# AIBluefisher/DReg-NeRF

Hardware: AMD Instinct MI355X
Metric: nerf_pairs_per_sec_regtr_fwd_bwd_128 (higher is better)
Workload: dtype bf16; 1 GPU; RegTR fwd+bwd+AdamW, shell-R synthetic pairs, 128^3 grids, 4 pairs (8 grids) per GPU per step, random-init weights; global_batch_pairs=4, resolution=128, fpn_head=active-set (identical results; rows around occupied voxels), parallelism=dp1

## Files before the change

dreg_nerf_amd/csrc/executor.hip:

```cpp
#include <hip/hip_runtime.h>
#include <cstdint>
#include <cstring>
#include <algorithm>
#include <vector>
#include <string>
#include <cstdio>
#include "../../include/dreg_nerf.h"
#ifndef DREG_ELAUNCH
#define DREG_ELAUNCH (-2)
#endif

namespace {

enum { OP_CONV = 0, OP_BN = 1, OP_MAXPOOL = 2, OP_CONV_ROWS = 3 };
constexpr int OP_INTS = 16;
constexpr int TENSOR_INTS = 5;
constexpr int RL = 8;
constexpr int PARAM_I64 = 5;

struct Tensor { int B, D, H, W, C; size_t bytes, off, goff; };
struct Param {
    float* val; float* grad; int d0, d1, ksz;
    size_t pk_fwd = SIZE_MAX, pk_dgrad = SIZE_MAX, pk_cls = SIZE_MAX;
    size_t pk_halo_fwd = SIZE_MAX, pk_halo_dgrad = SIZE_MAX;
    size_t pk_brick_fwd = SIZE_MAX, pk_brick_dgrad = SIZE_MAX;
    int cin_pad = 0;
};
struct Op {
    int kind, in, out, in2, w, b, p2, p3, p4, ksz, stride, pad, relu, add_same, rows_out, rows_in;
    size_t aux0 = 0, aux1 = 0;
    size_t wg_off = 0, wg_bytes = 0;
    int rd = -1;
    int ds_rows = -1;
    int sparse_gx = 0;
    size_t cl_off = 0;
    int cl_count = 0;
    int ds_sparse = 0;
    size_t cl2_off = 0;
    int cl2_count = 0;
    int pool = -1;
    int sstem = 0;
    int sstem_conv = -1, sstem_lat = -1;
    size_t xam_off = 0, pmask_off = 0;
    int halo = 0;
    int pointwise = 0;
    int stats_bn = -1;
    size_t stats_off = 0;
    int stats_conv = -1;
    int grp = 0;
    int fold_sk_fwd = 0, fold_sk_bwd = 0;
    int fold_into = -1, res_from = -1;
    int bt = -1;
    size_t keep_var = 0, keep_sums = 0;
};
struct HaloPack { const float* w; size_t off; int Cout, Cin, transposed, brick; };
struct PackRec { const float* w; void* out; int Cout, Cin_real, inner, ntaps, for_dgrad, Kpad, dtype, row0; };
static_assert(sizeof(PackRec) == 48, "matches PackDesc of conv.hip");

struct ReduceRec { const float* part; float* dw; int nsplit, Cout, Kpad, ntaps, Cin, Cin_real, accumulate, block0; };
static_assert(sizeof(ReduceRec) == 48, "matches WgradReduceDesc of conv.hip");

struct BnTailRec { const float* a; const float* b; float* o0; float* o1; int B, V, C, block0; };
static_assert(sizeof(BnTailRec) == 48, "matches BnTailDesc of fpn_ops.hip");

struct TimedLaunch { hipEvent_t e0, e1; int op, kind, variant; };

struct Exec {
    std::vector<Tensor> t;
    std::vector<Op> ops;
    std::vector<Param> prm;
    std::vector<char> needs_grad;
    size_t act_bytes = 0, arena_bytes = 0, pack_bytes = 0;
    size_t off_bn_ws = 0, off_coef = 0, off_ks = 0, off_rd = 0, off_cs = 0, off_tmp = 0;
    size_t sz_ks = 0;
    std::vector<ReduceRec> reduce;
    const void* sparse_arena = nullptr;
    std::vector<ReduceRec> reduce_abs;
    int reduce_blocks = 0;
    const void* reduce_arena = nullptr;
    std::vector<BnTailRec> bn_fwd, bn_bwd;
    size_t off_bnf = 0, off_bnb = 0;
    int bn_blocks = 0;
    std::vector<PackRec> packs;
    std::vector<HaloPack> halo_packs;
    int pack_rows = 0, pack_max_floats = 0;
    int out_slot = -1;
    bool timing = false;
    std::vector<TimedLaunch> timed;
    size_t timed_used = 0;
    hipStream_t aux = nullptr;
    std::vector<hipEvent_t> ev;
    hipEvent_t ev_done = nullptr;
    bool use_aux = true;
    const uint8_t* in_rowocc = nullptr;
    char* pack_base = nullptr;
    std::vector<char> written;
    bool aux_used = false;
    struct GrpLaunch { size_t off; int n, variant, blocks; };
    std::vector<int> grp_ops;
    std::vector<GrpLaunch> grp_launch;
    size_t off_grp = 0;
    bool grp_ready = false;
    int pend_sk_bn = -1, pend_sk_n = 0;
    size_t pend_sk_slice = 0;
    const void* fwd_rows_arena = nullptr;
    struct Band { size_t off; const char* tag; int idx; };
    std::vector<Band> bands;
    size_t off_guard_tab = 0, off_guard_res = 0;
    const void* guard_arena = nullptr;
    int guard_op = -1, guard_pass = 0; long long guard_band = -1;
    dreg_exec_opts opt;
};

inline size_t align256(size_t v) { return (v + 255) / 256 * 256; }
constexpr size_t GUARD_BYTES = 64 * 1024;
struct Bump {
    size_t v = 0;
    std::vector<Exec::Band>* bands = nullptr;
    const char* tag = "?"; int idx = -1;
    operator size_t() const { return v; }
    Bump& operator+=(size_t n) { v += n; if (bands && n) { bands->push_back(Exec::Band{v, tag, idx}); v += GUARD_BYTES; } return *this; }
    void name(const char* t, int i) { tag = t; idx = i; }
};
inline int out_dim(int i, int k, int s, int p) { return (i + 2 * p - k) / s + 1; }

struct Scope {
    Exec* e; hipStream_t st; TimedLaunch* tl = nullptr;
    Scope(Exec* ex, hipStream_t s, int op, int kind) : e(ex), st(s) {
        if (!e->timing) return;
        if (e->timed_used == e->timed.size()) {
            TimedLaunch n{}; n.op = op; n.kind = kind;
            if (hipEventCreate(&n.e0) != hipSuccess || hipEventCreate(&n.e1) != hipSuccess) return;
            e->timed.push_back(n);
        }
        tl = &e->timed[e->timed_used++];
        tl->op = op; tl->kind = kind; tl->variant = 0;
        (void)hipEventRecord(tl->e0, st);
    }
    ~Scope() { if (tl) (void)hipEventRecord(tl->e1, st); }
    void variant(int v) { if (tl) tl->variant = v; }
};

#define CK(expr) do { int rc_ = (expr); if (rc_) return rc_; } while (0)

bool s2_class_ok(const Param& p, int ksz, int stride, int pad)
{
    return stride == 2 && ((ksz == 3 && pad == 1) || (ksz == 1 && pad == 0)) && p.d0 % 64 == 0 && p.d1 % 64 == 0 && dreg_conv_get_glds();
}

}

extern "C" {

void dreg_exec_default_opts(dreg_exec_opts* o)
{
    std::memset(o, 0, sizeof(*o));
    o->sparse_grads = 1; o->bn_batch_tails = 1; o->fuse_stem = 1; o->sparse_stem = 1; o->fold_res_bn = 1; o->fold_splitk = 1;
    o->group_wgrad = 1; o->s2_accumulate = 1; o->fuse_bn_stats = 1; o->brick = 1; o->defer_head_pg = 0; o->pointwise_stream = 1;
}
void* dreg_exec_create(const int* tensors, int nt, const int* ops, int nops, const int64_t* params, int np)
{
    return dreg_exec_create_opts(tensors, nt, ops, nops, params, np, nullptr);
}
void* dreg_exec_create_opts(const int* tensors, int nt, const int* ops, int nops, const int64_t* params, int np, const dreg_exec_opts* opts)
{
    Exec* e = new Exec();
    if (opts) e->opt = *opts; else dreg_exec_default_opts(&e->opt);
    e->opt.brick &= 3;
    const int g_sparse_grads = e->opt.sparse_grads, g_bn_batch_tails = e->opt.bn_batch_tails, g_fuse_stem = e->opt.fuse_stem, g_sparse_stem = e->opt.sparse_stem,
              g_fold_res_bn = e->opt.fold_res_bn, g_fold_splitk = e->opt.fold_splitk, g_group_wgrad = e->opt.group_wgrad, g_fuse_bn_stats = e->opt.fuse_bn_stats,
              g_brick = e->opt.brick;
    e->t.resize(nt);
    for (int i = 0; i < nt; ++i) {
        Tensor& t = e->t[i];
        t.B = tensors[i * TENSOR_INTS]; t.D = tensors[i * TENSOR_INTS + 1]; t.H = tensors[i * TENSOR_INTS + 2];
        t.W = tensors[i * TENSOR_INTS + 3]; t.C = tensors[i * TENSOR_INTS + 4];
        t.bytes = align256((size_t)t.B * t.D * t.H * t.W * t.C * 2);
    }
    e->prm.resize(np);
    for (int i = 0; i < np; ++i) {
        Param& p = e->prm[i];
        p.val = (float*)params[i * PARAM_I64]; p.grad = (float*)params[i * PARAM_I64 + 1];
        p.d0 = (int)params[i * PARAM_I64 + 2]; p.d1 = (int)params[i * PARAM_I64 + 3]; p.ksz = (int)params[i * PARAM_I64 + 4];
    }
    e->ops.resize(nops);
    for (int i = 0; i < nops; ++i) {
        const int* r = ops + i * OP_INTS;
        Op& o = e->ops[i];
        o.kind = r[0]; o.in = r[1]; o.out = r[2]; o.in2 = r[3]; o.w = r[4]; o.b = r[5]; o.p2 = r[6]; o.p3 = r[7]; o.p4 = r[8];
        o.ksz = r[9]; o.stride = r[10]; o.pad = r[11]; o.relu = r[12]; o.add_same = r[13]; o.rows_out = r[14]; o.rows_in = r[15];
        if (o.in < 0 || o.in >= nt || o.out <= 0 || o.out >= nt || o.in2 >= nt) { delete e; return nullptr; }
    }
    e->out_slot = nops ? e->ops.back().out : -1;

    e->needs_grad.assign(nt, 0);
    for (const Op& o : e->ops) {
        bool g = e->needs_grad[o.in] || (o.in2 >= 0 && e->needs_grad[o.in2]);
        if (o.kind == OP_CONV || o.kind == OP_CONV_ROWS) g = g || e->prm[o.w].grad || (o.b >= 0 && e->prm[o.b].grad);
        if (o.kind == OP_BN) g = g || e->prm[o.w].grad || e->prm[o.b].grad;
        e->needs_grad[o.out] = g;
    }

    for (size_t i = 0; i + 1 < e->ops.size(); ++i) {
        Op& o = e->ops[i];
        if (o.kind != OP_BN || o.in2 >= 0 || o.out == e->out_slot) continue;
        int users = 0, pool = -1;
        for (size_t j = 0; j < e->ops.size(); ++j) {
            const Op& q = e->ops[j];
            if (q.in == o.out || q.in2 == o.out) { ++users; if (q.kind == OP_MAXPOOL && q.in == o.out && j > i) pool = (int)j; }
        }
        if (users == 1 && pool >= 0 && e->t[o.out].C % 8 == 0 && g_fuse_stem) { o.pool = pool; e->ops[pool].pool = (int)i; }
        if (o.pool < 0 && pool >= 0 && o.relu && e->t[o.out].C % 8 == 0 && g_sparse_stem && g_fuse_stem) {
            int prod = -1, writers = 0, lat = -1, others = 0;
            for (size_t j = 0; j < e->ops.size(); ++j) {
                const Op& q = e->ops[j];
                if (q.out == o.in) { prod = (int)j; ++writers; }
                if ((int)j == pool) continue;
                if (q.in2 == o.out) ++others;
                else if (q.in == o.out) { if (q.kind == OP_CONV_ROWS && q.rows_in >= 0 && lat < 0) lat = (int)j; else ++others; }
            }
            if (writers == 1 && others == 0 && e->ops[prod].kind == OP_CONV && e->ops[prod].rows_out >= 0 && o.b >= 0) {
                o.pool = pool; e->ops[pool].pool = (int)i; o.sstem = 1; o.sstem_conv = prod; o.sstem_lat = lat;
            }
        }
// ... 10 lines not shown
                if (o.in == bj.out) ++users;
                if (o.in2 == bj.out) { ++users; if (o.kind == OP_BN && q > j && o.pool < 0) k = (int)q; }
            }
            if (users != 1 || k < 0 || e->ops[k].res_from >= 0) continue;
            bj.fold_into = k; e->ops[k].res_from = (int)j;
        }

    if (g_fold_splitk)
        for (size_t i = 0; i < e->ops.size(); ++i) {
            Op& o = e->ops[i];
            if (o.kind != OP_CONV || o.b >= 0 || o.in2 >= 0 || o.relu || o.rows_out >= 0) continue;
            auto users = [&](int slot) { int u = 0; for (const Op& q : e->ops) u += (q.in == slot) + (q.in2 == slot); return u; };
            const Tensor& y = e->t[o.out];
            if (i + 1 < e->ops.size() && o.out != e->out_slot) {
                const Op& bn = e->ops[i + 1];
                if (bn.kind == OP_BN && bn.in == o.out && bn.pool < 0 && users(o.out) == 1 && dreg_bn_small_in_regs(y.B, y.D * y.H * y.W, y.C, 0)) o.fold_sk_fwd = 1;
            }
            const Tensor& x = e->t[o.in];
            if (i >= 1 && o.in != 0) {
                const Op& bn = e->ops[i - 1];
                if (bn.kind == OP_BN && bn.out == o.in && bn.pool < 0 && users(o.in) == 1 && dreg_bn_small_in_regs(x.B, x.D * x.H * x.W, x.C, 0) && o.stride == 1) o.fold_sk_bwd = 1;
            }
        }

    Bump off;
    if (e->opt.guard) { off.bands = &e->bands; off.name("arena start", 0); off += 256; }
    for (int i = 1; i < nt; ++i) { off.name("activation", i); e->t[i].off = off; off += e->t[i].bytes; }
    size_t max_tensor = 0, bn_ws = 0, coef = 0, cs = 0;
    for (Op& o : e->ops) {
        const Tensor& x = e->t[o.in];
        off.name(o.kind == OP_BN ? "BatchNorm statistics / stem scratch of op" : (o.kind == OP_MAXPOOL ? "max-pool argmax of op" : "conv op"), (int)(&o - e->ops.data()));
        if (o.kind == OP_BN) {
            const size_t sb = align256((size_t)x.B * x.C * 2 * sizeof(float));
            o.aux0 = off; off += sb; o.aux1 = off; off += sb;
            const size_t V = (size_t)x.D * x.H * x.W;
            size_t w = (size_t)x.B * dreg_bn_num_chunks((int)V) * x.C * 2 * sizeof(float);
            if (o.sstem) {
                const Tensor& p = e->t[e->ops[o.pool].out];
                const size_t w2 = dreg_sparse_stem_workspace_floats(p.B, p.D, p.H, p.W, p.C) * sizeof(float);
                if (w2 > w) w = w2;
                o.xam_off = off; off += align256((size_t)p.B * p.D * p.H * p.W * p.C * 2);
                o.pmask_off = off; off += align256((size_t)p.B * p.D * p.H * p.W);
            }
            if (w > bn_ws) bn_ws = w;
            if (sb > coef) coef = sb;
            bool shared = false;
            for (const Op& q : e->ops) shared = shared || (&q != &o && q.kind == OP_BN && (q.w == o.w || q.b == o.b || q.p2 == o.p2 || q.p3 == o.p3));
            if (g_bn_batch_tails && o.pool < 0 && !shared && dreg_bn_small(x.B, (int)V, x.C, 0)) {
                o.keep_var = off; off += align256((size_t)x.B * x.C * sizeof(float));
                o.keep_sums = off; off += sb;
                BnTailRec f{}, b{};
                f.a = (const float*)o.aux1; f.b = (const float*)o.keep_var; f.o0 = e->prm[o.p2].val; f.o1 = e->prm[o.p3].val;
                b.a = (const float*)o.keep_sums; b.b = nullptr; b.o0 = e->prm[o.w].grad; b.o1 = e->prm[o.b].grad;
                f.B = b.B = x.B; f.V = b.V = (int)V; f.C = b.C = x.C; f.block0 = b.block0 = e->bn_blocks;
                e->bn_blocks += (x.C + 255) / 256;
                o.bt = (int)e->bn_fwd.size();
                e->bn_fwd.push_back(f); e->bn_bwd.push_back(b);
            }
        } else if (o.kind == OP_MAXPOOL) {
            const Tensor& y = e->t[o.out];
            o.aux0 = off; off += align256((size_t)y.B * y.D * y.H * y.W * y.C);
        } else {
            const Param& w = e->prm[o.w];
            const Tensor& y = e->t[o.out];
            const size_t k1 = dreg_conv3d_igemm_workspace_bytes(x.B, x.D, x.H, x.W, x.C, y.D, y.H, y.W, w.d0, o.ksz, o.stride, o.pad, 0, o.in2 >= 0, 0);
            const size_t k2 = dreg_conv3d_igemm_workspace_bytes(x.B, y.D, y.H, y.W, w.d0, x.D, x.H, x.W, w.d1, o.ksz, o.stride, o.pad, 1, 0, 0);
            if (k1 > e->sz_ks) e->sz_ks = k1;
            if (k2 > e->sz_ks) e->sz_ks = k2;
            if (w.grad) {
                o.wg_bytes = dreg_conv3d_wgrad_workspace_bytes(x.B, y.D, y.H, y.W, x.C, w.d0, o.ksz, 0);
                bool shared = false;
                for (const ReduceRec& q : e->reduce) shared = shared || q.dw == w.grad;
                if (shared) o.rd = -2;
                else {
                    ReduceRec r{};
                    r.dw = w.grad; r.nsplit = dreg_conv3d_wgrad_splits(x.B, y.D, y.H, y.W, x.C, w.d0, o.ksz, 0);
                    r.Cout = w.d0; r.Kpad = dreg_conv3d_kpad(o.ksz, x.C, 0); r.ntaps = o.ksz * o.ksz * o.ksz; r.Cin = x.C; r.Cin_real = w.d1;
                    r.accumulate = (o.kind == OP_CONV_ROWS || o.rows_out >= 0) ? 3 : 1;
                    r.block0 = e->reduce_blocks;
                    e->reduce_blocks += dreg_wgrad_reduce_blocks(w.d0, w.d1, o.ksz, r.nsplit);
                    o.rd = (int)e->reduce.size();
                    e->reduce.push_back(r);
                }
            }
            const size_t c = dreg_colsum_workspace_bytes((size_t)y.B * y.D * y.H * y.W, w.d0);
            if (c > cs) cs = c;
        }
    }
    if (g_fuse_bn_stats) {
        for (size_t j = 0; j < e->ops.size(); ++j) {
            Op& bn = e->ops[j];
            if (bn.kind != OP_BN || bn.pool >= 0) continue;
            const Tensor& x = e->t[bn.in];
            const int V = x.D * x.H * x.W;
            if (V % 128 != 0 || dreg_bn_small(x.B, V, x.C, 0)) continue;
            int prod = -1, writers = 0;
            for (size_t i = 0; i < j; ++i) if (e->ops[i].out == bn.in) { prod = (int)i; ++writers; }
            if (writers != 1 || e->ops[prod].kind != OP_CONV || e->ops[prod].stats_bn >= 0) continue;
            {
                const Op& pc = e->ops[prod];
                const Tensor& px = e->t[pc.in];
                const Param& pp = e->prm[pc.w];
                if (!pc.relu && pp.d1 == px.C && pp.d0 != 64 && dreg_conv3_halo_use(px.B, px.D, px.H, px.W, px.C, pp.d0, pc.ksz, pc.stride, pc.pad)) continue;
            }
            e->ops[prod].stats_bn = (int)j;
            bn.stats_conv = prod;
// ... 128 lines not shown
        if (o.halo & 1) { if (p.pk_halo_fwd == SIZE_MAX) p.pk_halo_fwd = add_halo_pack(p, 0); }
        else if (p.pk_fwd == SIZE_MAX) { p.cin_pad = x.C; p.pk_fwd = add_pack(p, 0, x.C); }
        if (e->needs_grad[o.in]) {
            if (o.halo & 2) { if (p.pk_halo_dgrad == SIZE_MAX) p.pk_halo_dgrad = add_halo_pack(p, 1); }
            else if (o.kind == OP_CONV && s2_class_ok(p, o.ksz, o.stride, o.pad)) { if (p.pk_cls == SIZE_MAX) p.pk_cls = add_pack(p, 2, x.C); }
            else if (p.pk_dgrad == SIZE_MAX) p.pk_dgrad = add_pack(p, 1, x.C);
        }
    }
    e->pack_bytes = poff + 256;
    return e;
}

void dreg_exec_destroy(void* h)
{
    Exec* e = (Exec*)h;
    if (!e) return;
    for (auto& t : e->timed) { (void)hipEventDestroy(t.e0); (void)hipEventDestroy(t.e1); }
    for (auto& v : e->ev) if (v) (void)hipEventDestroy(v);
    if (e->ev_done) (void)hipEventDestroy(e->ev_done);
    delete e;
}

size_t dreg_exec_arena_bytes(void* h) { return ((Exec*)h)->arena_bytes; }
size_t dreg_exec_pack_bytes(void* h) { return ((Exec*)h)->pack_bytes; }
int dreg_exec_num_packs(void* h) { return (int)((Exec*)h)->packs.size(); }
size_t dreg_exec_tensor_offset(void* h, int slot) { return ((Exec*)h)->t[slot].off; }
int dreg_exec_output_slot(void* h) { return ((Exec*)h)->out_slot; }

int dreg_exec_pack_rows(void* h) { return ((Exec*)h)->pack_rows; }
int dreg_exec_export_pack_table(void* h, void* host_out, int* host_row_desc, void* pack_base)
{
    Exec* e = (Exec*)h;
    e->pack_base = (char*)pack_base;
    PackRec* o = (PackRec*)host_out;
    for (size_t i = 0; i < e->packs.size(); ++i) {
        o[i] = e->packs[i]; o[i].out = (char*)pack_base + (size_t)e->packs[i].out;
        const int end = i + 1 < e->packs.size() ? e->packs[i + 1].row0 : e->pack_rows;
        for (int r = e->packs[i].row0; r < end; ++r) host_row_desc[r] = (int)i;
    }
    return DREG_OK;
}
int dreg_exec_repack(void* h, const void* descs_dev, const int* row_desc_dev, void* stream)
{
    Exec* e = (Exec*)h;
    CK(dreg_pack_conv_weights_batched(descs_dev, (int)e->packs.size(), e->pack_rows, e->pack_max_floats, row_desc_dev, stream));
    for (const HaloPack& hp : e->halo_packs) {
        if (hp.brick) CK(dreg_pack_conv_weight_brick(hp.w, e->pack_base + hp.off, hp.Cout, hp.Cin, hp.transposed, stream));
        else CK(dreg_pack_conv_weight_halo(hp.w, e->pack_base + hp.off, hp.Cout, hp.Cin, hp.transposed, stream));
    }
    return DREG_OK;
}
int dreg_exec_op_halo(void* h, int op) { Exec* e = (Exec*)h; return op >= 0 && op < (int)e->ops.size() ? e->ops[op].halo : 0; }
int dreg_exec_op_wgrad_grouped(void* h, int op) { Exec* e = (Exec*)h; return op >= 0 && op < (int)e->ops.size() ? e->ops[op].grp : 0; }
int dreg_exec_op_pointwise(void* h, int op) { Exec* e = (Exec*)h; return op >= 0 && op < (int)e->ops.size() ? e->ops[op].pointwise : 0; }

void dreg_exec_set_overlap(void* h, int enable) { ((Exec*)h)->use_aux = enable != 0; }
void dreg_exec_set_input_row_occupancy(void* h, const uint8_t* rowocc) { ((Exec*)h)->in_rowocc = rowocc; }
void dreg_exec_set_timing(void* h, int enable) { ((Exec*)h)->timing = enable != 0; }
int dreg_exec_read_timings(void* h, int* op_kind, float* ms, int max)
{
    Exec* e = (Exec*)h;
    int n = 0;
    for (size_t i = 0; i < e->timed_used && n < max; ++i) {
        float v = 0.f;
        if (hipEventElapsedTime(&v, e->timed[i].e0, e->timed[i].e1) != hipSuccess) continue;
        op_kind[3 * n] = e->timed[i].op; op_kind[3 * n + 1] = e->timed[i].kind; op_kind[3 * n + 2] = e->timed[i].variant; ms[n] = v; ++n;
    }
    e->timed_used = 0;
    return n;
}

static int guard_setup(Exec* e, char* A, hipStream_t st)
{
    if (!e->opt.guard || e->guard_arena == (const void*)A) return DREG_OK;
    std::vector<unsigned long long> offs(e->bands.size());
    for (size_t i = 0; i < offs.size(); ++i) offs[i] = e->bands[i].off;
    if (!offs.empty() && hipMemcpyAsync(A + e->off_guard_tab, offs.data(), offs.size() * sizeof(unsigned long long), hipMemcpyHostToDevice, st) != hipSuccess) return DREG_ELAUNCH;
    if (hipStreamSynchronize(st) != hipSuccess) return DREG_ELAUNCH;
    int rc = dreg_guard_fill(A, A + e->off_guard_tab, (int)offs.size(), (int)GUARD_BYTES, (void*)st);
    if (rc) return rc;
    e->guard_arena = A;
    return DREG_OK;
}
static int guard_scan(Exec* e, char* A, long long* out4, hipStream_t st)
{
    int rc = dreg_guard_scan(A, A + e->off_guard_tab, (int)e->bands.size(), (int)GUARD_BYTES, A + e->off_guard_res, (void*)st);
    if (rc) return rc;
    if (hipMemcpyAsync(out4, A + e->off_guard_res, 4 * sizeof(long long), hipMemcpyDeviceToHost, st) != hipSuccess) return DREG_ELAUNCH;
    if (hipStreamSynchronize(st) != hipSuccess) return DREG_ELAUNCH;
    return DREG_OK;
}
static int guard_after_op(Exec* e, char* A, int op, int pass, hipStream_t st, hipStream_t aux)
{
    if (e->opt.guard < 2) return DREG_OK;
    if (aux && hipStreamSynchronize(aux) != hipSuccess) return DREG_ELAUNCH;
    long long r[4];
    int rc = guard_scan(e, A, r, st);
    if (rc) return rc;
    if (r[0] > 0) { e->guard_op = op; e->guard_pass = pass; e->guard_band = r[1]; return DREG_EGUARD; }
    return DREG_OK;
}
static int upload_tables(Exec* e, char* A, hipStream_t st)
{
    { int rc = guard_setup(e, A, st); if (rc) return rc; }
    if (e->reduce_arena == (const void*)A) return DREG_OK;
    e->reduce_abs = e->reduce;
    for (ReduceRec& r : e->reduce_abs) r.part = (const float*)(A + (size_t)r.part);
    std::vector<BnTailRec> f = e->bn_fwd, b = e->bn_bwd;
    for (BnTailRec& r : f) { r.a = (const float*)(A + (size_t)r.a); r.b = (const float*)(A + (size_t)r.b); }
    for (BnTailRec& r : b) r.a = (const float*)(A + (size_t)r.a);
    if (!e->reduce_abs.empty() && hipMemcpyAsync(A + e->off_rd, e->reduce_abs.data(), e->reduce_abs.size() * sizeof(ReduceRec), hipMemcpyHostToDevice, st) != hipSuccess) return DREG_ELAUNCH;
    if (!f.empty() && (hipMemcpyAsync(A + e->off_bnf, f.data(), f.size() * sizeof(BnTailRec), hipMemcpyHostToDevice, st) != hipSuccess ||
                       hipMemcpyAsync(A + e->off_bnb, b.data(), b.size() * sizeof(BnTailRec), hipMemcpyHostToDevice, st) != hipSuccess)) return DREG_ELAUNCH;
    const int gd = dreg_wgrad_group_desc_bytes();
    struct Rec { std::vector<char> d; int variant, nblocks, op; };
    std::vector<Rec> recs;
    e->grp_launch.clear(); e->grp_ready = false;
    bool all_ok = !e->grp_ops.empty();
    for (int i : e->grp_ops) {
        const Op& o = e->ops[i];
        const Tensor& x = e->t[o.in];
        const Tensor& y = e->t[o.out];
        const Param& w = e->prm[o.w];
        Rec r; r.d.resize(gd); r.op = i;
        if (e->t[o.out].goff == SIZE_MAX ||
            dreg_conv3d_wgrad_group_fill(r.d.data(), A + y.goff, A + x.off, A + o.wg_off, o.wg_bytes, x.B, x.D, x.H, x.W, x.C, y.D, y.H, y.W, w.d0,
                                         o.ksz, o.stride, o.pad, &r.variant, &r.nblocks) != DREG_OK || w.d1 != x.C) { all_ok = false; break; }
        recs.push_back(std::move(r));
    }
    std::vector<char> gtab;
    if (all_ok) {
        std::stable_sort(recs.begin(), recs.end(), [](const Rec& a, const Rec& b) { return a.variant < b.variant; });
        gtab.resize(recs.size() * (size_t)gd);
        for (size_t k = 0; k < recs.size(); ++k) {
            if (e->grp_launch.empty() || e->grp_launch.back().variant != recs[k].variant) e->grp_launch.push_back(Exec::GrpLaunch{e->off_grp + k * (size_t)gd, 0, recs[k].variant, 0});
            const int b0 = e->grp_launch.back().blocks;
            std::memcpy(recs[k].d.data() + gd - (int)sizeof(int), &b0, sizeof(int));
            std::memcpy(gtab.data() + k * (size_t)gd, recs[k].d.data(), (size_t)gd);
            e->grp_launch.back().n += 1; e->grp_launch.back().blocks += recs[k].nblocks;
        }
        if (hipMemcpyAsync(A + e->off_grp, gtab.data(), gtab.size(), hipMemcpyHostToDevice, st) != hipSuccess) return DREG_ELAUNCH;
        e->grp_ready = true;
    }
    if (hipStreamSynchronize(st) != hipSuccess) return DREG_ELAUNCH;
    e->reduce_arena = A;
    return DREG_OK;
}
static int flush_bn_tails(Exec* e, char* A, std::vector<char>& done, int what, hipStream_t st)
{
    for (int lo = 0, nrec = (int)done.size(); lo < nrec;) {
        if (!done[lo]) { ++lo; continue; }
        int hi = lo;
        while (hi + 1 < nrec && done[hi + 1]) ++hi;
        Scope sc(e, st, -1, 4 + what);
        const int b0 = e->bn_fwd[lo].block0;
        const int b1 = hi + 1 < nrec ? e->bn_fwd[hi + 1].block0 : e->bn_blocks;
        if (what == 0) CK(dreg_bn_running_update_batched((const BnTailRec*)(A + e->off_bnf) + lo, hi - lo + 1, b0, b1 - b0, 0.1f, (void*)st));
        else CK(dreg_bn_param_grad_batched((const BnTailRec*)(A + e->off_bnb) + lo, hi - lo + 1, b0, b1 - b0, 1, (void*)st));
        for (int q = lo; q <= hi; ++q) done[q] = 0;
        lo = hi + 1;
    }
    return DREG_OK;
}
// ... 74 lines not shown
                                           o.ksz, o.stride, o.pad, 0, o.relu, ta ? ta->D : 0, ta ? ta->H : 0, ta ? ta->W : 0, o.add_same,
                                           A + e->off_ks, e->sz_ks, o.in == 0 ? e->in_rowocc : nullptr, &ns, &sl, stream));
                if (ns > 0) { fwd_sk_bn = (int)i + 1; fwd_sk_n = ns; fwd_sk_slice = sl; }
                continue;
            }
            CK(dreg_conv3d_igemm_occ(act(o.in), PK + w.pk_fwd, act(o.out), bias, add, x.B, x.D, x.H, x.W, x.C, y.D, y.H, y.W, w.d0,
                                     o.ksz, o.stride, o.pad, 0, o.relu, ta ? ta->D : 0, ta ? ta->H : 0, ta ? ta->W : 0, o.add_same, 0, 0,
                                     A + e->off_ks, e->sz_ks, o.in == 0 ? e->in_rowocc : nullptr, stream));
        } else if (o.kind == OP_CONV_ROWS) {
            const Param& w = e->prm[o.w];
            if (o.rows_out < 0 || o.rows_out >= nlists) return DREG_EINVAL;
            const float* bias = o.b >= 0 ? e->prm[o.b].val : nullptr;
            const void* add = o.in2 >= 0 ? act(o.in2) : nullptr;
            const Tensor* ta = o.in2 >= 0 ? &e->t[o.in2] : nullptr;
            Scope sc(e, st, (int)i, 0);
            const int64_t* rl = rowlists + RL * o.rows_out;
            if ((e->opt.brick & (w.d0 == 64 ? 1 : 2)) && w.pk_brick_fwd != SIZE_MAX && rl[2] && rl[3] > 0) {
                sc.variant(2);
                CK(dreg_conv3_brick(act(o.in), PK + w.pk_brick_fwd, act(o.out), bias, add, (const void*)rl[2], (int)rl[3], (const int*)rl[4], (const void*)rl[5],
                                    (const int*)rl[6], x.B, x.D, x.H, x.W, x.C, w.d0, ta ? ta->D : 0, ta ? ta->H : 0, ta ? ta->W : 0, 0, 0, stream));
                continue;
            }
            CK(dreg_conv3d_igemm_rows(act(o.in), PK + w.pk_fwd, act(o.out), bias, add, (const int*)rl[0], (int)rl[1],
                                      x.B, x.D, x.H, x.W, x.C, y.D, y.H, y.W, w.d0, o.ksz, 1, o.pad, 0, 0, ta ? ta->D : 0, ta ? ta->H : 0, ta ? ta->W : 0,
                                      0, 0, stream));
        } else if (o.kind == OP_BN && o.pool >= 0 && o.sstem) {
            const Op& q = e->ops[o.pool];
            const Tensor& p = e->t[q.out];
            const Op& cv = e->ops[o.sstem_conv];
            if (cv.rows_out >= nlists) return DREG_EINVAL;
            const int64_t* rl = rowlists + RL * cv.rows_out;
            const int* ra = nullptr; int na = 0;
            if (o.sstem_lat >= 0) {
                const int li = e->ops[o.sstem_lat].rows_in;
                if (li < 0 || li >= nlists) return DREG_EINVAL;
                ra = (const int*)rowlists[RL * li]; na = (int)rowlists[RL * li + 1];
            }
            CK(dreg_sparse_stem_fwd(act(o.in), (const int*)rl[0], (int)rl[1], ra, na, act(o.out), act(q.out), (uint8_t*)(A + q.aux0), A + o.xam_off, (uint8_t*)(A + o.pmask_off),
                                    e->prm[o.w].val, e->prm[o.b].val, e->prm[o.p2].val, e->prm[o.p3].val, (float*)(A + o.aux0), (float*)(A + o.aux1),
                                    (float*)(A + e->off_bn_ws), x.B, x.D, x.H, x.W, p.D, p.H, p.W, x.C, 1e-5f, 0.1f, train, o.relu, stream));
        } else if (o.kind == OP_BN && o.pool >= 0) {
            const Op& q = e->ops[o.pool];
            const Tensor& p = e->t[q.out];
            CK(dreg_bn_relu_maxpool_fwd(act(o.in), act(q.out), (uint8_t*)(A + q.aux0), e->prm[o.w].val, e->prm[o.b].val, e->prm[o.p2].val, e->prm[o.p3].val,
                                        (float*)(A + o.aux0), (float*)(A + o.aux1), (float*)(A + e->off_bn_ws), x.B, x.D, x.H, x.W, p.D, p.H, p.W, x.C,
                                        1e-5f, 0.1f, train, o.relu, stream));
        } else if (o.kind == OP_MAXPOOL && o.pool >= 0) {
        } else if (o.kind == OP_BN) {
            const int V = x.D * x.H * x.W;
            const void* res_p = o.in2 >= 0 ? act(o.in2) : nullptr;
            void* out_p = o.fold_into >= 0 ? nullptr : act(o.out);
            dreg_bn_extra ex{};
            if (o.res_from >= 0) { res_p = act(e->ops[o.res_from].in); ex.res_scale_shift = (const float*)(A + e->ops[o.res_from].aux0); }
            if (train && sums_rpc[i] > 0) {
                CK(dreg_bn3d_fwd_ex(act(o.in), res_p, out_p, e->prm[o.w].val, e->prm[o.b].val, e->prm[o.p2].val, e->prm[o.p3].val,
                                    (float*)(A + o.aux0), (float*)(A + o.aux1), (float*)(A + o.stats_off), x.B, V, x.C, 1e-5f, 0.1f, 1, o.relu, 0,
                                    nullptr, nullptr, sums_rpc[i], &ex, stream));
                continue;
            }
            int deferred = 0;
            if (fwd_sk_bn == (int)i) { ex.splitk_part = (const float*)(A + e->off_ks); ex.splitk_nsplit = fwd_sk_n; ex.splitk_slice = fwd_sk_slice; fwd_sk_bn = -1; }
            CK(dreg_bn3d_fwd_ex(act(o.in), res_p, out_p, e->prm[o.w].val, e->prm[o.b].val, e->prm[o.p2].val, e->prm[o.p3].val,
                                (float*)(A + o.aux0), (float*)(A + o.aux1), (float*)(A + e->off_bn_ws), x.B, V, x.C, 1e-5f, 0.1f, train, o.relu, 0,
                                o.bt >= 0 ? (float*)(A + o.keep_var) : nullptr, &deferred, 0, &ex, stream));
            if (deferred) bn_done[o.bt] = 1;
        } else if (o.kind == OP_MAXPOOL) {
            CK(dreg_maxpool3d_fwd(act(o.in), act(o.out), (uint8_t*)(A + o.aux0), x.B, x.D, x.H, x.W, y.D, y.H, y.W, x.C, 0, stream));
        } else return DREG_EINVAL;
    }
    CK(guard_after_op(e, A, (int)e->ops.size() - 1, 0, st, nullptr));
    CK(flush_bn_tails(e, A, bn_done, 0, st));
    CK(guard_after_op(e, A, (int)e->ops.size(), 0, st, nullptr));
    arena_mark.ok = true;
    return DREG_OK;
}
int dreg_exec_guard_bands(void* h) { return (int)((Exec*)h)->bands.size(); }
int dreg_exec_guard_check(void* h, void* arena, long long* out4, void* stream)
{
    Exec* e = (Exec*)h;
    if (!e->opt.guard || !out4) return DREG_EINVAL;
    if (e->guard_arena != arena) { out4[0] = 0; out4[1] = (long long)e->bands.size(); out4[2] = 0; out4[3] = 0; return DREG_OK; }
    return guard_scan(e, (char*)arena, out4, (hipStream_t)stream);
}
int dreg_exec_guard_describe(void* h, int band, char* buf, int buf_bytes)
{
    Exec* e = (Exec*)h;
    if (band < 0 || band >= (int)e->bands.size() || !buf || buf_bytes <= 0) return DREG_EINVAL;
    const Exec::Band& b = e->bands[band];
    std::snprintf(buf, (size_t)buf_bytes, "band %d at arena offset %zu, behind: %s %d", band, b.off, b.tag, b.idx);
    return DREG_OK;
}
int dreg_exec_guard_last(void* h, int* op, int* pass, long long* band)
{
    Exec* e = (Exec*)h;
    if (op) *op = e->guard_op;
    if (pass) *pass = e->guard_pass;
    if (band) *band = e->guard_band;
    return DREG_OK;
}

int dreg_exec_backward_range(void* h, void* arena, size_t arena_bytes, const void* pack_base, const void* x_in, const void* grad_out,
                             const int64_t* rowlists, int nlists, void* stream, void* aux_stream, int op_begin, int op_end, int flags);
int dreg_exec_backward(void* h, void* arena, size_t arena_bytes, const void* pack_base, const void* x_in, const void* grad_out,
                       const int64_t* rowlists, int nlists, void* stream, void* aux_stream)
{
    return dreg_exec_backward_range(h, arena, arena_bytes, pack_base, x_in, grad_out, rowlists, nlists, stream, aux_stream,
                                    0, (int)((Exec*)h)->ops.size(), 3);
}
int dreg_exec_backward_range(void* h, void* arena, size_t arena_bytes, const void* pack_base, const void* x_in, const void* grad_out,
                             const int64_t* rowlists, int nlists, void* stream, void* aux_stream, int op_begin, int op_end, int flags)
{
    Exec* e = (Exec*)h;
    if (arena_bytes < e->arena_bytes || op_begin < 0 || op_end > (int)e->ops.size() || op_begin > op_end) return DREG_EINVAL;
    char* A = (char*)arena;
    const char* PK = (const char*)pack_base;
    hipStream_t st = (hipStream_t)stream;
    auto act = [&](int s) -> void* { return s == 0 ? (void*)x_in : (void*)(A + e->t[s].off); };
// ... 216 lines not shown
                    else
                    CK(dreg_conv3d_igemm_ws(gy, PK + w.pk_dgrad, gx, nullptr, gx, x.B, y.D, y.H, y.W, w.d0, x.D, x.H, x.W, w.d1,
                                            o.ksz, o.stride, o.pad, 1, 0, x.D, x.H, x.W, 1, 0, 0, A + e->off_ks, e->sz_ks, stream));
                } else if (rows) {
                    if (o.rows_in < 0 || o.rows_in >= nlists) return DREG_EINVAL;
                    const int64_t* rl = rowlists + RL * o.rows_in;
                    const int* r_in = (const int*)rl[0];
                    const int n_in = (int)rl[1];
                    if (o.sparse_gx && gx == grad(o.in)) {
                        if (n_in > 0 && hipMemcpyAsync(A + o.cl_off, r_in, (size_t)n_in * sizeof(int), hipMemcpyDeviceToDevice, st) != hipSuccess) return DREG_ELAUNCH;
                        const_cast<Op&>(o).cl_count = n_in;
                    } else CK(dreg_fill_zero(gx, (size_t)x.B * x.D * x.H * x.W * x.C * 2, stream));
                    if ((g_brick & (w.d1 == 64 ? 1 : 2)) && w.pk_brick_dgrad != SIZE_MAX && rl[2] && rl[3] > 0) {
                        sc.variant(2);
                        CK(dreg_conv3_brick(gy, PK + w.pk_brick_dgrad, gx, nullptr, nullptr, (const void*)rl[2], (int)rl[3], (const int*)rl[4], (const void*)rl[5],
                                            (const int*)rl[6], x.B, x.D, x.H, x.W, w.d0, w.d1, 0, 0, 0, 0, 0, stream));
                    } else
                        CK(dreg_conv3d_igemm_rows(gy, PK + w.pk_dgrad, gx, nullptr, nullptr, r_in, n_in,
                                                  x.B, y.D, y.H, y.W, w.d0, x.D, x.H, x.W, x.C, o.ksz, 1, o.pad, 1, 0, 0, 0, 0, 0, 0, stream));
                } else if (w.pk_cls != SIZE_MAX && s2_class_ok(w, o.ksz, o.stride, o.pad)) {
                    CK(dreg_conv3d_dgrad_s2(gy, PK + w.pk_cls, gx, x.B, x.D, x.H, x.W, x.C, y.D, y.H, y.W, w.d0, o.ksz, o.pad, stream));
                } else {
                    if (w.pk_dgrad == SIZE_MAX) return DREG_EINVAL;
                    if (o.fold_sk_bwd && gx == grad(o.in) && i - 1 >= 0) {
                        int ns = 0; size_t sl = 0;
                        CK(dreg_conv3d_igemm_defer(gy, PK + w.pk_dgrad, gx, nullptr, nullptr, x.B, y.D, y.H, y.W, w.d0, x.D, x.H, x.W, w.d1,
                                                   o.ksz, o.stride, o.pad, 1, 0, 0, 0, 0, 0, A + e->off_ks, e->sz_ks, nullptr, &ns, &sl, stream));
                        if (ns > 0) { e->pend_sk_bn = i - 1; e->pend_sk_n = ns; e->pend_sk_slice = sl; }
                    } else if (o.pointwise & 2)
                        CK(dreg_conv1_stream(gy, PK + w.pk_dgrad, gx, nullptr, nullptr, x.B, y.D, y.H, y.W, w.d0, x.D, x.H, x.W, w.d1,
                                             o.ksz, o.stride, o.pad, 1, 0, 0, 0, 0, 0, 0, 0, A + e->off_ks, e->sz_ks, stream, 0));
                    else
                    CK(dreg_conv3d_igemm_ws(gy, PK + w.pk_dgrad, gx, nullptr, nullptr, x.B, y.D, y.H, y.W, w.d0, x.D, x.H, x.W, w.d1,
                                            o.ksz, o.stride, o.pad, 1, 0, 0, 0, 0, 0, 0, 0, A + e->off_ks, e->sz_ks, stream));
                }
            }
            if (e->needs_grad[o.in] && !fused_add) CK(commit(o.in));
        } else if (o.kind == OP_BN) {
            const int V = x.D * x.H * x.W;
            const bool res_g = o.in2 >= 0 && e->needs_grad[o.in2];
            void* dx = dst_for(o.in);
            void* dres = nullptr;
            bool res_via_copy = false;
            if (res_g) {
                if (!written[o.in2]) dres = grad(o.in2);
                else if (dx != (void*)(A + e->off_tmp)) dres = A + e->off_tmp;
                else res_via_copy = true;
            }
            if (!e->prm[o.w].grad || !e->prm[o.b].grad) return DREG_EINVAL;
            int deferred = 0;
            if (res_via_copy) {
                CK(dreg_bn3d_bwd_defer_params(act(o.in), gy, act(o.out), (float*)(A + o.aux0), (float*)(A + o.aux1), dx, nullptr, e->prm[o.w].grad, e->prm[o.b].grad,
                                              (float*)(A + e->off_coef), (float*)(A + e->off_bn_ws), x.B, V, x.C, o.relu, 1, 0,
                                              o.bt >= 0 ? (float*)(A + o.keep_sums) : nullptr, &deferred, stream));
                if (deferred) bn_done[o.bt] = 1;
                CK(commit(o.in));
                if (o.relu) CK(dreg_relu_bwd(act(o.out), gy, A + e->off_tmp, (size_t)x.B * V * x.C, 0, 0, 0, stream));
                else if (hipMemcpyAsync(A + e->off_tmp, gy, (size_t)x.B * V * x.C * 2, hipMemcpyDeviceToDevice, st) != hipSuccess) return DREG_ELAUNCH;
                CK(commit(o.in2));
            } else {
                dreg_bn_extra ex{};
                if (e->pend_sk_bn == i) { ex.splitk_part = (const float*)(A + e->off_ks); ex.splitk_nsplit = e->pend_sk_n; ex.splitk_slice = e->pend_sk_slice; e->pend_sk_bn = -1; }
                CK(dreg_bn3d_bwd_ex(act(o.in), gy, o.in2 >= 0 ? act(o.out) : nullptr, (float*)(A + o.aux0), (float*)(A + o.aux1), dx, dres, e->prm[o.w].grad, e->prm[o.b].grad,
                                    (float*)(A + e->off_coef), (float*)(A + e->off_bn_ws), x.B, V, x.C, o.relu, 1, 0,
                                    o.bt >= 0 ? (float*)(A + o.keep_sums) : nullptr, &deferred, &ex, stream));
                if (deferred) bn_done[o.bt] = 1;
                if (res_g && dres == (void*)(A + e->off_tmp)) { CK(commit(o.in2)); CK(commit(o.in)); }
                else { CK(commit(o.in)); if (res_g) CK(commit(o.in2)); }
            }
        } else if (o.kind == OP_MAXPOOL) {
            if (!e->needs_grad[o.in]) continue;
            CK(dreg_maxpool3d_bwd_acc(gy, (const uint8_t*)(A + o.aux0), grad(o.in), x.B, x.D, x.H, x.W, y.D, y.H, y.W, x.C, written[o.in] ? 1 : 0, 0, stream));
            written[o.in] = 1;
        }
    }
    CK(guard_after_op(e, A, op_begin, 1, st, aux_on ? e->aux : nullptr));
    CK(run_deferred());
    if (!grp_seen.empty()) CK(flush_group(e->grp_ops.front()));
    CK(flush_reduce());
    CK(flush_bn_tails(e, A, bn_done, 1, st));
    CK(guard_after_op(e, A, -1, 1, st, aux_on ? e->aux : nullptr));
    if ((flags & 2) && aux_used) {
        if (hipEventRecord(e->ev_done, e->aux) != hipSuccess || hipStreamWaitEvent(st, e->ev_done, 0) != hipSuccess) return DREG_ELAUNCH;
    }
    return DREG_OK;
}

}
```

dreg_nerf_amd/csrc/fpn_ops.hip:

```cpp
#include "common.h"
#include "../../include/dreg_nerf.h"
extern "C" int dreg_fill_zero(void* p, size_t bytes, void* stream);

template <typename T> struct Gran;
template <> struct Gran<float> {
    static constexpr int G = 4;
    static __device__ __forceinline__ void ld(const float* p, float (&v)[4]) { float4 q = *reinterpret_cast<const float4*>(p); v[0] = q.x; v[1] = q.y; v[2] = q.z; v[3] = q.w; }
    static __device__ __forceinline__ void st(float* p, const float (&v)[4]) { *reinterpret_cast<float4*>(p) = make_float4(v[0], v[1], v[2], v[3]); }
    static __device__ __forceinline__ void unpack(const uint4& q, float (&v)[4]) { v[0] = __uint_as_float(q.x); v[1] = __uint_as_float(q.y); v[2] = __uint_as_float(q.z); v[3] = __uint_as_float(q.w); }
    static __device__ __forceinline__ uint4 pack(const float (&v)[4]) { return make_uint4(__float_as_uint(v[0]), __float_as_uint(v[1]), __float_as_uint(v[2]), __float_as_uint(v[3])); }
};
template <> struct Gran<bf16_t> {
    static constexpr int G = 8;
    static __device__ __forceinline__ void ld(const bf16_t* p, float (&v)[8]) {
        uint4 q = *reinterpret_cast<const uint4*>(p);
        uint32_t w[4] = {q.x, q.y, q.z, q.w};
#pragma unroll
        for (int i = 0; i < 4; ++i) { v[2 * i] = __uint_as_float(w[i] << 16); v[2 * i + 1] = __uint_as_float(w[i] & 0xffff0000u); }
    }
    static __device__ __forceinline__ void st(bf16_t* p, const float (&v)[8]) {
        uint32_t w[4];
#pragma unroll
        for (int i = 0; i < 4; ++i) w[i] = f2bf2(v[2 * i], v[2 * i + 1]);
        *reinterpret_cast<uint4*>(p) = make_uint4(w[0], w[1], w[2], w[3]);
// ... 63 lines not shown
    }
    if (r0 < rpi) {
        constexpr int UN = 4;
        for (int v = v0 + r0; v < v1; v += rpi * UN) {
            float xv[UN][G], gv[UN][G], yv[UN][G];
#pragma unroll
            for (int u = 0; u < UN; ++u)
                if (v + u * rpi < v1) {
                    const size_t off = ((size_t)b * V + v + u * rpi) * C + (size_t)cg * G;
                    Gran<T>::ld(x + off, xv[u]);
                    if (MODE == 1) {
                        Gran<T>::ld(dy + off, gv[u]);
                        if (relu && !remask) Gran<T>::ld(y + off, yv[u]);
                    }
                }
#pragma unroll
            for (int u = 0; u < UN; ++u)
                if (v + u * rpi < v1) {
                    if (MODE == 0) {
#pragma unroll
                        for (int i = 0; i < G; ++i) { s1[i] += xv[u][i]; s2[i] += xv[u][i] * xv[u][i]; }
                    } else {
                        if (remask) {
#pragma unroll
                            for (int i = 0; i < G; ++i) gv[u][i] = (xv[u][i] * sc[i] + sh[i]) > 0.f ? gv[u][i] : 0.f;
                        } else if (relu) {
#pragma unroll
                            for (int i = 0; i < G; ++i) gv[u][i] = yv[u][i] > 0.f ? gv[u][i] : 0.f;
                        }
                        if (gout) Gran<T>::st(gout + ((size_t)b * V + v + u * rpi) * C + (size_t)cg * G, gv[u]);
#pragma unroll
                        for (int i = 0; i < G; ++i) { s1[i] += gv[u][i]; s2[i] += gv[u][i] * (xv[u][i] - mu[i]) * rs[i]; }
                    }
                }
        }
    }
    __shared__ float red[256][2 * 8 + 1];
#pragma unroll
    for (int i = 0; i < G; ++i) { red[t][i] = s1[i]; red[t][G + i] = s2[i]; }
    __syncthreads();
    if (t < cgs) {
        float a1[G], a2[G];
#pragma unroll
        for (int i = 0; i < G; ++i) { a1[i] = 0.f; a2[i] = 0.f; }
        for (int r = 0; r < rpi; ++r)
#pragma unroll
            for (int i = 0; i < G; ++i) { a1[i] += red[r * cgs + t][i]; a2[i] += red[r * cgs + t][G + i]; }
        float* dst = partial + (((size_t)b * nchunks + chunk) * C + (size_t)cg * G) * 2;
#pragma unroll
        for (int i = 0; i < G; ++i) { dst[2 * i] = a1[i]; dst[2 * i + 1] = a2[i]; }
    }
}

constexpr int BN_MAX_GRIDS = 256;
__global__ __launch_bounds__(512) void bn_finalize_kernel(const float* __restrict__ partial, const float* __restrict__ gamma, const float* __restrict__ beta,
                                   float* __restrict__ running_mean, float* __restrict__ running_var,
                                   float* __restrict__ scale_shift, float* __restrict__ mean_rstd,
                                   int B, int nchunks, int C, int V, float eps, float momentum, int train)
{
    const int c = blockIdx.x, wave = threadIdx.x >> 6, lane = threadIdx.x & 63, nw = blockDim.x >> 6;
    const float ga = gamma[c], be = beta[c];
    if (!train) {
        const float rstd = 1.0f / sqrtf(running_var[c] + eps);
        for (int b = threadIdx.x; b < B; b += blockDim.x) {
            scale_shift[((size_t)b * C + c) * 2] = ga * rstd;
            scale_shift[((size_t)b * C + c) * 2 + 1] = be - running_mean[c] * ga * rstd;
            mean_rstd[((size_t)b * C + c) * 2] = running_mean[c];
            mean_rstd[((size_t)b * C + c) * 2 + 1] = rstd;
        }
        return;
    }
    __shared__ double stat[BN_MAX_GRIDS][2];
    for (int b = wave; b < B; b += nw) {
        double s1 = 0.0, s2 = 0.0;
#pragma unroll 8
        for (int k = lane; k < nchunks; k += 64) {
            const float2 p = *reinterpret_cast<const float2*>(partial + (((size_t)b * nchunks + k) * C + c) * 2);
            s1 += p.x; s2 += p.y;
        }
        s1 = wave_sum_d(s1); s2 = wave_sum_d(s2);
        const double mean = s1 / V;
        double var = s2 / V - mean * mean;
        if (var < 0) var = 0;
        if (lane == 0) {
            const float rstd = 1.0f / sqrtf((float)var + eps);
            scale_shift[((size_t)b * C + c) * 2] = ga * rstd;
            scale_shift[((size_t)b * C + c) * 2 + 1] = be - (float)mean * ga * rstd;
            mean_rstd[((size_t)b * C + c) * 2] = (float)mean;
            mean_rstd[((size_t)b * C + c) * 2 + 1] = rstd;
            stat[b][0] = mean; stat[b][1] = var;
        }
    }
    __syncthreads();
    if (threadIdx.x == 0) {
        float rm = running_mean[c], rv = running_var[c];
        for (int b = 0; b < B; ++b) {
            const double mean = stat[b][0], var = stat[b][1];
            const float unbiased = V > 1 ? (float)(var * V / (V - 1)) : (float)var;
            rm = (1.f - momentum) * rm + momentum * (float)mean;
            rv = (1.f - momentum) * rv + momentum * unbiased;
        }
        running_mean[c] = rm; running_var[c] = rv;
    }
}

template <typename T>
__global__ void bn_apply_kernel(const T* __restrict__ x, const float* __restrict__ scale_shift, const T* __restrict__ res,
                                T* __restrict__ y, size_t total_gran, int V, int C, int relu)
{
    constexpr int G = Gran<T>::G;
    const int CG = C / G;
    for (size_t i = blockIdx.x * (size_t)blockDim.x + threadIdx.x; i < total_gran; i += (size_t)gridDim.x * blockDim.x) {
        const int cg = (int)(i % CG);
        const int b = (int)((i / CG) / V);
        float xv[G], rv[G];
        Gran<T>::ld(x + i * G, xv);
        if (res) Gran<T>::ld(res + i * G, rv);
        const float* ss = scale_shift + ((size_t)b * C + (size_t)cg * G) * 2;
#pragma unroll
        for (int k = 0; k < G; ++k) {
            float v = xv[k] * ss[2 * k] + ss[2 * k + 1];
            if (res) v += rv[k];
            xv[k] = relu ? fmaxf(v, 0.f) : v;
        }
        Gran<T>::st(y + i * G, xv);
    }
}

__global__ __launch_bounds__(512) void bn_bwd_finalize_kernel(const float* __restrict__ partial, float* __restrict__ coef, float* __restrict__ dgamma,
                                       float* __restrict__ dbeta, int B, int nchunks, int C, int V, int accumulate)
{
    const int c = blockIdx.x, wave = threadIdx.x >> 6, lane = threadIdx.x & 63, nw = blockDim.x >> 6;
    __shared__ double stat[BN_MAX_GRIDS][2];
    for (int b = wave; b < B; b += nw) {
        double s1 = 0.0, s2 = 0.0;
#pragma unroll 8
        for (int k = lane; k < nchunks; k += 64) {
            const float2 p = *reinterpret_cast<const float2*>(partial + (((size_t)b * nchunks + k) * C + c) * 2);
            s1 += p.x; s2 += p.y;
        }
        s1 = wave_sum_d(s1); s2 = wave_sum_d(s2);
        if (lane == 0) {
            coef[((size_t)b * C + c) * 2] = (float)(s1 / V);
            coef[((size_t)b * C + c) * 2 + 1] = (float)(s2 / V);
            stat[b][0] = s1; stat[b][1] = s2;
        }
    }
    __syncthreads();
    if (threadIdx.x == 0) {
        double dg = 0.0, db = 0.0;
        for (int b = 0; b < B; ++b) { db += stat[b][0]; dg += stat[b][1]; }
        dgamma[c] = accumulate ? dgamma[c] + (float)dg : (float)dg;
        dbeta[c] = accumulate ? dbeta[c] + (float)db : (float)db;
    }
}

template <typename T>
__global__ void bn_bwd_apply_kernel(const T* __restrict__ x, const T* __restrict__ dy, const T* __restrict__ y,
                                    const float* __restrict__ mean_rstd, const float* __restrict__ scale_shift,
                                    const float* __restrict__ coef, T* __restrict__ dx, T* __restrict__ dres,
                                    size_t total_gran, int V, int C, int relu)
{
    constexpr int G = Gran<T>::G;
    const int CG = C / G;
    for (size_t i = blockIdx.x * (size_t)blockDim.x + threadIdx.x; i < total_gran; i += (size_t)gridDim.x * blockDim.x) {
        const int cg = (int)(i % CG);
        const int b = (int)((i / CG) / V);
        float xv[G], gv[G], yv[G];
        Gran<T>::ld(x + i * G, xv);
        Gran<T>::ld(dy + i * G, gv);
        const size_t pc = ((size_t)b * C + (size_t)cg * G) * 2;
        if (relu && y == nullptr) {
#pragma unroll
            for (int k = 0; k < G; ++k) gv[k] = (xv[k] * scale_shift[pc + 2 * k] + scale_shift[pc + 2 * k + 1]) > 0.f ? gv[k] : 0.f;
        } else if (relu) { Gran<T>::ld(y + i * G, yv);
#pragma unroll
            for (int k = 0; k < G; ++k) gv[k] = yv[k] > 0.f ? gv[k] : 0.f; }
        if (dres) Gran<T>::st(dres + i * G, gv);
#pragma unroll
        for (int k = 0; k < G; ++k) {
            const float xh = (xv[k] - mean_rstd[pc + 2 * k]) * mean_rstd[pc + 2 * k + 1];
            xv[k] = scale_shift[pc + 2 * k] * (gv[k] - coef[pc + 2 * k] - xh * coef[pc + 2 * k + 1]);
        }
        Gran<T>::st(dx + i * G, xv);
    }
}

template <typename T, int UN>
__global__ __launch_bounds__(256) void bn_apply_cols_kernel(const T* __restrict__ x, const float* __restrict__ scale_shift, const T* __restrict__ res,
                                                            T* __restrict__ y, int V, int C, int rows_per_chunk, int relu,
                                                            const float* __restrict__ res_ss = nullptr)
{
    constexpr int G = Gran<T>::G;
    const int CG = C / G, cgs = CG < 256 ? CG : 256, rpi = 256 / cgs;
    const int t = threadIdx.x, cg = blockIdx.z * cgs + (t % cgs), r0 = t / cgs, b = blockIdx.y;
    if (r0 >= rpi || cg >= CG) return;
    const int v0 = blockIdx.x * rows_per_chunk, v1 = min(v0 + rows_per_chunk, V);
    float sc[G], sh[G], rsc[G], rsh[G];
#pragma unroll
    for (int i = 0; i < G; ++i) {
        sc[i] = scale_shift[((size_t)b * C + cg * G + i) * 2]; sh[i] = scale_shift[((size_t)b * C + cg * G + i) * 2 + 1];
        if (res_ss) { rsc[i] = res_ss[((size_t)b * C + cg * G + i) * 2]; rsh[i] = res_ss[((size_t)b * C + cg * G + i) * 2 + 1]; }
    }
    for (int v = v0 + r0; v < v1; v += rpi * UN) {
        float xv[UN][G], rv[UN][G];
#pragma unroll
        for (int u = 0; u < UN; ++u)
            if (v + u * rpi < v1) {
                const size_t off = ((size_t)b * V + v + u * rpi) * C + (size_t)cg * G;
                Gran<T>::ld(x + off, xv[u]);
                if (res) Gran<T>::ld(res + off, rv[u]);
            }
#pragma unroll
        for (int u = 0; u < UN; ++u)
            if (v + u * rpi < v1) {
#pragma unroll
                for (int k = 0; k < G; ++k) {
                    float o = xv[u][k] * sc[k] + sh[k];
                    if (res) {
                        float r = rv[u][k];
                        if (res_ss) { r = r * rsc[k] + rsh[k]; if constexpr (sizeof(T) == 2) r = bf2f(f2bf(r)); }
                        o += r;
                    }
                    xv[u][k] = relu ? fmaxf(o, 0.f) : o;
                }
                Gran<T>::st(y + ((size_t)b * V + v + u * rpi) * C + (size_t)cg * G, xv[u]);
            }
    }
}
template <typename T, int UN>
__global__ __launch_bounds__(256) void bn_bwd_apply_cols_kernel(const T* __restrict__ x, const T* dy, const T* __restrict__ y,
                                                                const float* __restrict__ mean_rstd, const float* __restrict__ scale_shift,
                                                                const float* __restrict__ coef, T* __restrict__ dx, T* dres,
                                                                int V, int C, int rows_per_chunk, int relu, int g_stored = 0)
{
    constexpr int G = Gran<T>::G;
    const int CG = C / G, cgs = CG < 256 ? CG : 256, rpi = 256 / cgs;
    const int t = threadIdx.x, cg = blockIdx.z * cgs + (t % cgs), r0 = t / cgs, b = blockIdx.y;
    if (r0 >= rpi || cg >= CG) return;
    if (g_stored) { dy = dres; dres = nullptr; relu = 0; }
    const int v0 = blockIdx.x * rows_per_chunk, v1 = min(v0 + rows_per_chunk, V);
    float mu[G], rs[G], sc[G], sh[G], c1[G], c2[G];
#pragma unroll
    for (int i = 0; i < G; ++i) {
        const size_t pc = ((size_t)b * C + cg * G + i) * 2;
        mu[i] = mean_rstd[pc]; rs[i] = mean_rstd[pc + 1]; sc[i] = scale_shift[pc]; sh[i] = scale_shift[pc + 1]; c1[i] = coef[pc]; c2[i] = coef[pc + 1];
    }
    const bool remask = relu && y == nullptr;
    for (int v = v0 + r0; v < v1; v += rpi * UN) {
        float xv[UN][G], gv[UN][G], yv[UN][G];
#pragma unroll
        for (int u = 0; u < UN; ++u)
            if (v + u * rpi < v1) {
                const size_t off = ((size_t)b * V + v + u * rpi) * C + (size_t)cg * G;
                Gran<T>::ld(x + off, xv[u]);
                Gran<T>::ld(dy + off, gv[u]);
                if (relu && !remask) Gran<T>::ld(y + off, yv[u]);
            }
#pragma unroll
        for (int u = 0; u < UN; ++u)
            if (v + u * rpi < v1) {
                const size_t off = ((size_t)b * V + v + u * rpi) * C + (size_t)cg * G;
                if (remask) {
#pragma unroll
                    for (int k = 0; k < G; ++k) gv[u][k] = (xv[u][k] * sc[k] + sh[k]) > 0.f ? gv[u][k] : 0.f;
                } else if (relu) {
#pragma unroll
                    for (int k = 0; k < G; ++k) gv[u][k] = yv[u][k] > 0.f ? gv[u][k] : 0.f;
                }
                if (dres) Gran<T>::st(dres + off, gv[u]);
#pragma unroll
                for (int k = 0; k < G; ++k) {
                    const float xh = (xv[u][k] - mu[k]) * rs[k];
                    xv[u][k] = sc[k] * (gv[u][k] - c1[k] - xh * c2[k]);
                }
                Gran<T>::st(dx + off, xv[u]);
            }
    }
}

constexpr int BNS_COLS = 4, BNS_ROWS = 64;
template <int G> __device__ __forceinline__ void bns_reduce(float (&s1)[G], float (&s2)[G], float (*red)[BNS_COLS][16], int t)
{
#pragma unroll
    for (int o = 4; o < 64; o <<= 1)
#pragma unroll
        for (int i = 0; i < G; ++i) { s1[i] += __shfl_xor(s1[i], o, 64); s2[i] += __shfl_xor(s2[i], o, 64); }
    const int lane = t & 63, wave = t >> 6;
    if (lane < BNS_COLS) {
#pragma unroll
        for (int i = 0; i < G; ++i) { red[wave][lane][i] = s1[i]; red[wave][lane][8 + i] = s2[i]; }
    }
}
template <typename T>
__device__ __forceinline__ uint4 bns_sum_slices(const float* __restrict__ part, int nsplit, size_t slice, size_t off)
{
    constexpr int G = Gran<T>::G;
    float v[G];
#pragma unroll
    for (int i = 0; i < G; ++i) v[i] = 0.f;
#pragma unroll 4
    for (int sp = 0; sp < nsplit; ++sp) {
        const float* p = part + (size_t)sp * slice + off;
        const float4 a = *reinterpret_cast<const float4*>(p);
        v[0] += a.x; v[1] += a.y; v[2] += a.z; v[3] += a.w;
        if constexpr (G == 8) { const float4 b = *reinterpret_cast<const float4*>(p + 4); v[4] += b.x; v[5] += b.y; v[6] += b.z; v[7] += b.w; }
    }
    return Gran<T>::pack(v);
}
template <typename T, int NR = 0>
__global__ __launch_bounds__(256) void bn_small_fwd_kernel(const T* __restrict__ x, const T* __restrict__ res, T* __restrict__ y,
                                                           const float* __restrict__ gamma, const float* __restrict__ beta,
                                                           float* __restrict__ scale_shift, float* __restrict__ mean_rstd, float* __restrict__ var_out,
                                                           int V, int C, float eps, int relu,
                                                           const float* __restrict__ part = nullptr, int nsplit = 0, size_t slice = 0)
{
    constexpr int G = Gran<T>::G;
    const int t = threadIdx.x, col = t & (BNS_COLS - 1), rl = t >> 2, b = blockIdx.y;
    const int c0 = (blockIdx.x * BNS_COLS + col) * G;
    __shared__ float red[4][BNS_COLS][16];
    __shared__ float s_sc[BNS_COLS * 8], s_sh[BNS_COLS * 8];
    float s1[G], s2[G];
#pragma unroll
    for (int i = 0; i < G; ++i) s1[i] = s2[i] = 0.f;
    constexpr int NRR = NR > 0 ? NR : 1;
    uint4 xr[NRR], rr[NRR];
    if constexpr (NR > 0) {
#pragma unroll
        for (int j = 0; j < NR; ++j) {
            const size_t off = ((size_t)b * V + rl + j * BNS_ROWS) * C + c0;
            if (part) { xr[j] = bns_sum_slices<T>(part, nsplit, slice, off); *reinterpret_cast<uint4*>(const_cast<T*>(x) + off) = xr[j]; }
// ... 180 lines not shown
            Gran<T>::st(dx + off, xv);
        }
        return;
    }
#pragma unroll 4
    for (int v = rl; v < V; v += BNS_ROWS) {
        const size_t off = ((size_t)b * V + v) * C + c0;
        float xv[G], gv[G], yv[G];
        Gran<T>::ld(x + off, xv);
        Gran<T>::ld(dy + off, gv);
        if (relu && !remask) Gran<T>::ld(y + off, yv);
#pragma unroll
        for (int i = 0; i < G; ++i) {
            if (remask) gv[i] = (xv[i] * sc[i] + sh[i]) > 0.f ? gv[i] : 0.f;
            else if (relu) gv[i] = yv[i] > 0.f ? gv[i] : 0.f;
        }
        if (dres) Gran<T>::st(dres + off, gv);
#pragma unroll
        for (int i = 0; i < G; ++i) {
            const float xh = (xv[i] - mu[i]) * rs[i];
            xv[i] = sc[i] * (gv[i] - c1[i] - xh * c2[i]);
        }
        Gran<T>::st(dx + off, xv);
    }
}
__global__ void bn_param_grad_kernel(const float* __restrict__ sums, float* __restrict__ dgamma, float* __restrict__ dbeta, int B, int C, int accumulate)
{
    const int c = blockIdx.x * blockDim.x + threadIdx.x;
    if (c >= C) return;
    double db = 0.0, dg = 0.0;
    for (int b = 0; b < B; ++b) { db += sums[((size_t)b * C + c) * 2]; dg += sums[((size_t)b * C + c) * 2 + 1]; }
    dgamma[c] = accumulate ? dgamma[c] + (float)dg : (float)dg;
    dbeta[c] = accumulate ? dbeta[c] + (float)db : (float)db;
}
struct BnTailDesc {
    const float* a;
    const float* b;
    float* o0; float* o1;
    int B, V, C, block0;
};
static_assert(sizeof(BnTailDesc) == 48, "descriptor layout is part of the ABI");
template <int WHAT>
__global__ void bn_tail_batched_kernel(const BnTailDesc* __restrict__ descs, int n, int block_base, float momentum, int accumulate)
{
    const int blk = (int)blockIdx.x + block_base;
    int lo = 0, hi = n - 1;
    while (lo < hi) {
        const int mid = (lo + hi + 1) >> 1;
        if (descs[mid].block0 <= blk) lo = mid; else hi = mid - 1;
    }
    const BnTailDesc d = descs[lo];
    const int c = (blk - d.block0) * blockDim.x + threadIdx.x;
    if (c >= d.C) return;
    if (WHAT == 0) {
        float rm = d.o0[c], rv = d.o1[c];
        for (int b = 0; b < d.B; ++b) {
            const float mean = d.a[((size_t)b * d.C + c) * 2], vb = d.b[(size_t)b * d.C + c];
            const float unbiased = d.V > 1 ? (float)((double)vb * d.V / (d.V - 1)) : vb;
            rm = (1.f - momentum) * rm + momentum * mean;
            rv = (1.f - momentum) * rv + momentum * unbiased;
        }
        d.o0[c] = rm; d.o1[c] = rv;
    } else {
        double db = 0.0, dg = 0.0;
        for (int b = 0; b < d.B; ++b) { db += d.a[((size_t)b * d.C + c) * 2]; dg += d.a[((size_t)b * d.C + c) * 2 + 1]; }
        d.o0[c] = accumulate ? d.o0[c] + (float)dg : (float)dg;
        d.o1[c] = accumulate ? d.o1[c] + (float)db : (float)db;
    }
}
DREG_KNOB(int, g_bn_small_regs, 1);
DREG_KNOB(int, g_bn_store_g, 1);
DREG_KNOB(int, g_bn_debug_skip, 0);
DREG_KNOB(int, g_bn_small_maxv, 512);
static inline bool bn_small_ok(int B, int V, int C, int G) { return V >= 2 && V <= g_bn_small_maxv && C % (BNS_COLS * G) == 0 && B >= 1; }

template <typename T>
__global__ void maxpool_fwd_kernel(const T* __restrict__ x, T* __restrict__ y, uint8_t* __restrict__ arg,
                                   int B, int Di, int Hi, int Wi, int Do, int Ho, int Wo, int C)
{
    constexpr int G = Gran<T>::G;
    const int CG = C / G;
    const size_t total = (size_t)B * Do * Ho * Wo * CG;
    for (size_t i = blockIdx.x * (size_t)blockDim.x + threadIdx.x; i < total; i += (size_t)gridDim.x * blockDim.x) {
        int cg, ox, oy, oz, b;
        decode_gxyzb(i, CG, Wo, Ho, Do, cg, ox, oy, oz, b);
        float best[G];
        int bi[G];
#pragma unroll
        for (int k = 0; k < G; ++k) { best[k] = -INFINITY; bi[k] = 0; }
        for (int dz = 0; dz < 3; ++dz) {
            const int z = oz * 2 - 1 + dz; if ((unsigned)z >= (unsigned)Di) continue;
            for (int dy = 0; dy < 3; ++dy) {
                const int yy = oy * 2 - 1 + dy; if ((unsigned)yy >= (unsigned)Hi) continue;
                for (int dx = 0; dx < 3; ++dx) {
                    const int xx = ox * 2 - 1 + dx; if ((unsigned)xx >= (unsigned)Wi) continue;
                    float v[G];
                    Gran<T>::ld(x + ((((size_t)b * Di + z) * Hi + yy) * Wi + xx) * C + (size_t)cg * G, v);
                    const int tap = (dz * 3 + dy) * 3 + dx;
#pragma unroll
                    for (int k = 0; k < G; ++k) if (v[k] > best[k]) { best[k] = v[k]; bi[k] = tap; }
                }
            }
        }
        Gran<T>::st(y + i * G, best);
#pragma unroll
        for (int k = 0; k < G; ++k) arg[i * G + k] = (uint8_t)bi[k];
// ... 1016 lines not shown
        if (dl) lq = *reinterpret_cast<const uint4*>(dl + off);
        const int oz0 = iz >> 1, oy0 = iy >> 1, ox0 = ix >> 1;
        uint4 gq[8];
        uint2 aq[8];
        bool ok[8];
        int tp[8];
#pragma unroll
        for (int u = 0; u < 8; ++u) {
            const int uz = u >> 2, uy = (u >> 1) & 1, ux = u & 1;
            const int oz = oz0 + uz, oy = oy0 + uy, ox = ox0 + ux;
            ok[u] = (!uz || (iz & 1)) && (!uy || (iy & 1)) && (!ux || (ix & 1)) && oz < Do && oy < Ho && ox < Wo;
            tp[u] = ((iz - 2 * oz + 1) * 3 + (iy - 2 * oy + 1)) * 3 + (ix - 2 * ox + 1);
            if (ok[u]) {
                const size_t o = ((((size_t)b * Do + oz) * Ho + oy) * Wo + ox) * C + (size_t)cg * G;
                gq[u] = *reinterpret_cast<const uint4*>(dp + o);
                aq[u] = *reinterpret_cast<const uint2*>(arg + o);
            }
        }
        float xv[G], g[G], lv[G];
        Gran<bf16_t>::unpack(xq, xv);
#pragma unroll
        for (int k = 0; k < G; ++k) g[k] = 0.f;
#pragma unroll
        for (int u = 0; u < 8; ++u)
            if (ok[u]) {
                float gg[G];
                Gran<bf16_t>::unpack(gq[u], gg);
#pragma unroll
                for (int k = 0; k < G; ++k) {
                    const uint32_t a = ((k < 4 ? aq[u].x : aq[u].y) >> (8 * (k & 3))) & 0xffu;
                    if ((int)a == tp[u]) g[k] += gg[k];
                }
            }
        if (dl) {
            Gran<bf16_t>::unpack(lq, lv);
#pragma unroll
            for (int k = 0; k < G; ++k) g[k] += lv[k];
        }
#pragma unroll
        for (int k = 0; k < G; ++k) {
            if (relu && !((xv[k] * sc[k] + sh[k]) > 0.f)) g[k] = 0.f;
            const float xh = (xv[k] - mu[k]) * rs[k];
            xv[k] = sc[k] * (g[k] - c1[k] - xh * c2[k]);
        }
        Gran<bf16_t>::st(dx + off, xv);
    }
}

static inline int nblocks(size_t total, int per = 256, int cap = 8192) {
    size_t b = (total + per - 1) / per;
    return (int)(b > (size_t)cap ? cap : (b ? b : 1));
}
static inline bool slabs_ragged(int CG) { return CG > 256 && CG % 256 != 0; }
static inline int bn_rows_per_chunk(int V) { return V >= 262144 ? 512 : V >= 32768 ? 256 : V >= 4096 ? 128 : V >= 512 ? 32 : (V >= 8 ? 8 : V); }

extern "C" {

#ifdef DREG_PROBE
void dreg_bn_set_debug_skip(int mask) { g_bn_debug_skip = mask; }
void dreg_bn_set_store_g(int enable) { g_bn_store_g = enable ? 1 : 0; }
void dreg_bn_set_small_regs(int enable) { g_bn_small_regs = enable ? 1 : 0; }
void dreg_bn_set_small_max_voxels(int v) { g_bn_small_maxv = v; }
#endif
int dreg_bn_num_chunks(int V) { const int r = bn_rows_per_chunk(V); return (V + r - 1) / r; }

static int bn3d_fwd_impl(const void* x, const void* res, void* y, const float* gamma, const float* beta,
                         float* running_mean, float* running_var, float* scale_shift, float* mean_rstd, float* workspace,
                         int B, int V, int C, float eps, float momentum, int train, int relu, int dtype, void* stream, float* var_keep, int* deferred,
                         int sums_rows_per_chunk = 0, const dreg_bn_extra* ex = nullptr);
int dreg_bn3d_fwd(const void* x, const void* res, void* y, const float* gamma, const float* beta,
                  float* running_mean, float* running_var, float* scale_shift, float* mean_rstd, float* workspace,
                  int B, int V, int C, float eps, float momentum, int train, int relu, int dtype, void* stream)
{
    return bn3d_fwd_impl(x, res, y, gamma, beta, running_mean, running_var, scale_shift, mean_rstd, workspace, B, V, C, eps, momentum, train, relu, dtype, stream, nullptr, nullptr);
}
int dreg_bn3d_fwd_defer_update(const void* x, const void* res, void* y, const float* gamma, const float* beta,
                               float* running_mean, float* running_var, float* scale_shift, float* mean_rstd, float* workspace,
                               int B, int V, int C, float eps, float momentum, int train, int relu, int dtype, float* var_keep, int* deferred, void* stream)
{
    return bn3d_fwd_impl(x, res, y, gamma, beta, running_mean, running_var, scale_shift, mean_rstd, workspace, B, V, C, eps, momentum, train, relu, dtype, stream, var_keep, deferred);
}
int dreg_bn3d_fwd_from_sums(const void* x, const void* res, void* y, const float* gamma, const float* beta,
                            float* running_mean, float* running_var, float* scale_shift, float* mean_rstd, float* sums,
                            int rows_per_chunk, int B, int V, int C, float eps, float momentum, int relu, int dtype, void* stream)
{
    if (rows_per_chunk <= 0) return DREG_EINVAL;
    return bn3d_fwd_impl(x, res, y, gamma, beta, running_mean, running_var, scale_shift, mean_rstd, sums, B, V, C, eps, momentum, 1, relu, dtype, stream, nullptr, nullptr,
                         rows_per_chunk);
}
int dreg_bn3d_fwd_ex(const void* x, const void* res, void* y, const float* gamma, const float* beta,
                     float* running_mean, float* running_var, float* scale_shift, float* mean_rstd, float* workspace,
                     int B, int V, int C, float eps, float momentum, int train, int relu, int dtype, float* var_keep, int* deferred,
                     int sums_rows_per_chunk, const dreg_bn_extra* ex, void* stream)
{
    if (sums_rows_per_chunk < 0) return DREG_EINVAL;
    return bn3d_fwd_impl(x, res, y, gamma, beta, running_mean, running_var, scale_shift, mean_rstd, workspace, B, V, C, eps, momentum,
                         sums_rows_per_chunk > 0 ? 1 : train, relu, dtype, stream, var_keep, deferred, sums_rows_per_chunk, ex);
}
int dreg_bn_small(int B, int V, int C, int dtype) { return bn_small_ok(B, V, C, dtype == 0 ? 8 : 4) ? 1 : 0; }
int dreg_bn_running_update_batched(const void* descs_dev, int n, int block_base, int nblocks, float momentum, void* stream)
{
    if (n <= 0 || nblocks <= 0) return DREG_OK;
    hipLaunchKernelGGL(bn_tail_batched_kernel<0>, dim3(nblocks), dim3(256), 0, (hipStream_t)stream, (const BnTailDesc*)descs_dev, n, block_base, momentum, 0);
    DREG_LAUNCH_CHECK();
    return DREG_OK;
}
int dreg_bn_param_grad_batched(const void* descs_dev, int n, int block_base, int nblocks, int accumulate, void* stream)
{
    if (n <= 0 || nblocks <= 0) return DREG_OK;
    hipLaunchKernelGGL(bn_tail_batched_kernel<1>, dim3(nblocks), dim3(256), 0, (hipStream_t)stream, (const BnTailDesc*)descs_dev, n, block_base, 0.f, accumulate);
    DREG_LAUNCH_CHECK();
    return DREG_OK;
}
struct BnSplitkIn { const float* part = nullptr; int nsplit = 0; size_t slice = 0; };
int dreg_bn_small_in_regs(int B, int V, int C, int dtype)
{
    return (g_bn_small_regs && bn_small_ok(B, V, C, dtype == 0 ? 8 : 4) && (V == 8 * BNS_ROWS || V == BNS_ROWS)) ? 1 : 0;
}
static int bn3d_fwd_impl(const void* x, const void* res, void* y, const float* gamma, const float* beta,
                         float* running_mean, float* running_var, float* scale_shift, float* mean_rstd, float* workspace,
                         int B, int V, int C, float eps, float momentum, int train, int relu, int dtype, void* stream, float* var_keep, int* deferred,
                         int sums_rows_per_chunk, const dreg_bn_extra* ex)
{
    hipStream_t st = (hipStream_t)stream;
    const float* res_ss = ex ? ex->res_scale_shift : nullptr;
    BnSplitkIn ski;
    if (ex) { ski.part = ex->splitk_part; ski.nsplit = ex->splitk_nsplit; ski.slice = ex->splitk_slice; }
    if (ski.part && !(train && sums_rows_per_chunk == 0 && dreg_bn_small_in_regs(B, V, C, dtype))) return DREG_EINVAL;
    if (deferred) *deferred = 0;
    const int G = dtype == 0 ? 8 : 4;
    if (C % G) return DREG_EINVAL;
    const int rpc = bn_rows_per_chunk(V), nch = (V + rpc - 1) / rpc;
    const int CG = C / G, slabs = (CG + 255) / 256;
    const bool presummed = train && sums_rows_per_chunk > 0;
    if (presummed && V % sums_rows_per_chunk != 0) return DREG_EINVAL;
    if (train && !presummed && bn_small_ok(B, V, C, G)) {
        if (res_ss || !y) return DREG_EINVAL;
        const dim3 g1(CG / BNS_COLS, B);
        float* var = var_keep ? var_keep : workspace;
#define BNS_FWD(Tt, NRv) hipLaunchKernelGGL((bn_small_fwd_kernel<Tt, NRv>), g1, dim3(256), 0, st, (const Tt*)x, (const Tt*)res, (Tt*)y, gamma, beta, \
                                            scale_shift, mean_rstd, var, V, C, eps, relu, ski.part, ski.nsplit, ski.slice)
        const int nr = !g_bn_small_regs ? 0 : (V == 8 * BNS_ROWS ? 8 : (V == BNS_ROWS ? 1 : 0));
        if (dtype == 0) { if (nr == 8) BNS_FWD(bf16_t, 8); else if (nr == 1) BNS_FWD(bf16_t, 1); else BNS_FWD(bf16_t, 0); }
        else { if (nr == 8) BNS_FWD(float, 8); else if (nr == 1) BNS_FWD(float, 1); else BNS_FWD(float, 0); }
#undef BNS_FWD
        DREG_LAUNCH_CHECK();
        if (var_keep && deferred) { *deferred = 1; return DREG_OK; }
        hipLaunchKernelGGL(bn_running_update_kernel, dim3((C + 255) / 256), dim3(256), 0, st, mean_rstd, var, running_mean, running_var, B, V, C, momentum);
        DREG_LAUNCH_CHECK();
        return DREG_OK;
    }
    if (train && V < 2) return DREG_EINVAL;
    if (B > BN_MAX_GRIDS || (train && !presummed && slabs_ragged(CG))) return DREG_EINVAL;
    if (train && !presummed && !(g_bn_debug_skip & 1)) {
        dim3 grid(nch, B, slabs);
        if (dtype == 0) hipLaunchKernelGGL((bn_partial_kernel<bf16_t, 0>), grid, dim3(256), 0, st, (const bf16_t*)x, nullptr, nullptr, nullptr, workspace, V, C, rpc, 0);
        else hipLaunchKernelGGL((bn_partial_kernel<float, 0>), grid, dim3(256), 0, st, (const float*)x, nullptr, nullptr, nullptr, workspace, V, C, rpc, 0);
        DREG_LAUNCH_CHECK();
    }
    hipLaunchKernelGGL(bn_finalize_kernel, dim3(C), dim3(64 * (B < 8 ? B : 8)), 0, st, workspace, gamma, beta, running_mean, running_var,
                       scale_shift, mean_rstd, B, presummed ? V / sums_rows_per_chunk : nch, C, V, eps, momentum, train);
    DREG_LAUNCH_CHECK();
    if (!y) return DREG_OK;
    const dim3 agrid(nch, B, slabs);
    if (dtype == 0) hipLaunchKernelGGL((bn_apply_cols_kernel<bf16_t, 4>), agrid, dim3(256), 0, st, (const bf16_t*)x, scale_shift, (const bf16_t*)res, (bf16_t*)y, V, C, rpc, relu, res ? res_ss : nullptr);
    else hipLaunchKernelGGL((bn_apply_cols_kernel<float, 4>), agrid, dim3(256), 0, st, (const float*)x, scale_shift, (const float*)res, (float*)y, V, C, rpc, relu, res ? res_ss : nullptr);
    DREG_LAUNCH_CHECK();
    return DREG_OK;
}

static int bn3d_bwd_impl(const void* x, const void* dy, const void* y, const float* scale_shift, const float* mean_rstd,
                         void* dx, void* dres, float* dgamma, float* dbeta, float* coef, float* workspace,
                         int B, int V, int C, int relu, int accumulate, int dtype, void* stream, float* sums_keep, int* deferred, const dreg_bn_extra* ex = nullptr);
int dreg_bn3d_bwd(const void* x, const void* dy, const void* y, const float* scale_shift, const float* mean_rstd,
                  void* dx, void* dres, float* dgamma, float* dbeta, float* coef, float* workspace,
                  int B, int V, int C, int relu, int accumulate, int dtype, void* stream)
{
    return bn3d_bwd_impl(x, dy, y, scale_shift, mean_rstd, dx, dres, dgamma, dbeta, coef, workspace, B, V, C, relu, accumulate, dtype, stream, nullptr, nullptr);
}
int dreg_bn3d_bwd_defer_params(const void* x, const void* dy, const void* y, const float* scale_shift, const float* mean_rstd,
                               void* dx, void* dres, float* dgamma, float* dbeta, float* coef, float* workspace,
                               int B, int V, int C, int relu, int accumulate, int dtype, float* sums_keep, int* deferred, void* stream)
{
    return bn3d_bwd_impl(x, dy, y, scale_shift, mean_rstd, dx, dres, dgamma, dbeta, coef, workspace, B, V, C, relu, accumulate, dtype, stream, sums_keep, deferred);
}
int dreg_bn3d_bwd_ex(const void* x, const void* dy, const void* y, const float* scale_shift, const float* mean_rstd,
                     void* dx, void* dres, float* dgamma, float* dbeta, float* coef, float* workspace,
                     int B, int V, int C, int relu, int accumulate, int dtype, float* sums_keep, int* deferred, const dreg_bn_extra* ex, void* stream)
{
    return bn3d_bwd_impl(x, dy, y, scale_shift, mean_rstd, dx, dres, dgamma, dbeta, coef, workspace, B, V, C, relu, accumulate, dtype, stream, sums_keep, deferred, ex);
}
static int bn3d_bwd_impl(const void* x, const void* dy, const void* y, const float* scale_shift, const float* mean_rstd,
                         void* dx, void* dres, float* dgamma, float* dbeta, float* coef, float* workspace,
                         int B, int V, int C, int relu, int accumulate, int dtype, void* stream, float* sums_keep, int* deferred, const dreg_bn_extra* ex)
{
    hipStream_t st = (hipStream_t)stream;
    BnSplitkIn ski;
    if (ex) { ski.part = ex->splitk_part; ski.nsplit = ex->splitk_nsplit; ski.slice = ex->splitk_slice; }
    if (ski.part && !dreg_bn_small_in_regs(B, V, C, dtype)) return DREG_EINVAL;
    if (deferred) *deferred = 0;
    const int G = dtype == 0 ? 8 : 4;
    if (C % G) return DREG_EINVAL;
    const int rpc = bn_rows_per_chunk(V), nch = (V + rpc - 1) / rpc;
    const int CG = C / G, slabs = (CG + 255) / 256;
    if (bn_small_ok(B, V, C, G)) {
        const dim3 g1(CG / BNS_COLS, B);
        float* sums = sums_keep ? sums_keep : coef;
#define BNS_BWD(Tt, NRv) hipLaunchKernelGGL((bn_small_bwd_kernel<Tt, NRv>), g1, dim3(256), 0, st, (const Tt*)x, (const Tt*)dy, (const Tt*)y, scale_shift, mean_rstd, \
                                            (Tt*)dx, (Tt*)dres, sums, V, C, relu, ski.part, ski.nsplit, ski.slice)
        const int nr = !g_bn_small_regs ? 0 : (V == 8 * BNS_ROWS ? 8 : (V == BNS_ROWS ? 1 : 0));
        if (dtype == 0) { if (nr == 8) BNS_BWD(bf16_t, 8); else if (nr == 1) BNS_BWD(bf16_t, 1); else BNS_BWD(bf16_t, 0); }
        else { if (nr == 8) BNS_BWD(float, 8); else if (nr == 1) BNS_BWD(float, 1); else BNS_BWD(float, 0); }
#undef BNS_BWD
        DREG_LAUNCH_CHECK();
        if (sums_keep && deferred) { *deferred = 1; return DREG_OK; }
        hipLaunchKernelGGL(bn_param_grad_kernel, dim3((C + 255) / 256), dim3(256), 0, st, sums, dgamma, dbeta, B, C, accumulate);
        DREG_LAUNCH_CHECK();
        return DREG_OK;
    }
    if (B > BN_MAX_GRIDS || slabs_ragged(CG)) return DREG_EINVAL;
    dim3 grid(nch, B, slabs);
    const int g_stored = (dres && relu && y && dres != dy && dres != dx && g_bn_store_g && !(g_bn_debug_skip & 2)) ? 1 : 0;
    if (g_bn_debug_skip & 2) {}
    else if (dtype == 0) hipLaunchKernelGGL((bn_partial_kernel<bf16_t, 1>), grid, dim3(256), 0, st, (const bf16_t*)x, (const bf16_t*)dy, (const bf16_t*)y, mean_rstd, workspace, V, C, rpc, relu, scale_shift, g_stored ? (bf16_t*)dres : nullptr);
    else hipLaunchKernelGGL((bn_partial_kernel<float, 1>), grid, dim3(256), 0, st, (const float*)x, (const float*)dy, (const float*)y, mean_rstd, workspace, V, C, rpc, relu, scale_shift, g_stored ? (float*)dres : nullptr);
    DREG_LAUNCH_CHECK();
    hipLaunchKernelGGL(bn_bwd_finalize_kernel, dim3(C), dim3(64 * (B < 8 ? B : 8)), 0, st, workspace, coef, dgamma, dbeta, B, nch, C, V, accumulate);
    DREG_LAUNCH_CHECK();
    const size_t tg = (size_t)B * V * CG;
    (void)tg;
    if (dtype == 0) hipLaunchKernelGGL((bn_bwd_apply_cols_kernel<bf16_t, 4>), grid, dim3(256), 0, st, (const bf16_t*)x, (const bf16_t*)dy, (const bf16_t*)y, mean_rstd, scale_shift, coef, (bf16_t*)dx, (bf16_t*)dres, V, C, rpc, relu, g_stored);
    else hipLaunchKernelGGL((bn_bwd_apply_cols_kernel<float, 4>), grid, dim3(256), 0, st, (const float*)x, (const float*)dy, (const float*)y, mean_rstd, scale_shift, coef, (float*)dx, (float*)dres, V, C, rpc, relu, g_stored);
    DREG_LAUNCH_CHECK();
    return DREG_OK;
}

int dreg_bn_relu_maxpool_fwd(const void* x, void* pooled, uint8_t* argmax, const float* gamma, const float* beta,
                             float* running_mean, float* running_var, float* scale_shift, float* mean_rstd, float* workspace,
                             int B, int Di, int Hi, int Wi, int Do, int Ho, int Wo, int C, float eps, float momentum, int train, int relu, void* stream)
{
    hipStream_t st = (hipStream_t)stream;
    const int V = Di * Hi * Wi;
    if (C % 8 || B > BN_MAX_GRIDS || (train && V < 2)) return DREG_EINVAL;
    const int rpc = bn_rows_per_chunk(V), nch = (V + rpc - 1) / rpc;
    const int CG = C / 8, slabs = (CG + 255) / 256;
    if (train && slabs_ragged(CG)) return DREG_EINVAL;
    if (train) {
        hipLaunchKernelGGL((bn_partial_kernel<bf16_t, 0>), dim3(nch, B, slabs), dim3(256), 0, st, (const bf16_t*)x, nullptr, nullptr, nullptr, workspace, V, C, rpc, 0);
        DREG_LAUNCH_CHECK();
    }
    hipLaunchKernelGGL(bn_finalize_kernel, dim3(C), dim3(64 * (B < 8 ? B : 8)), 0, st, workspace, gamma, beta, running_mean, running_var,
                       scale_shift, mean_rstd, B, nch, C, V, eps, momentum, train);
    DREG_LAUNCH_CHECK();
    const size_t total = (size_t)B * Do * Ho * Wo * CG;
    hipLaunchKernelGGL(bn_relu_maxpool_fwd_kernel<bf16_t>, dim3(nblocks(total)), dim3(256), 0, st, (const bf16_t*)x, scale_shift, (bf16_t*)pooled, argmax,
                       B, Di, Hi, Wi, Do, Ho, Wo, C, relu);
    DREG_LAUNCH_CHECK();
    return DREG_OK;
}
int dreg_bn_relu_maxpool_bwd(const void* x, const void* dp, const uint8_t* argmax, const float* scale_shift, const float* mean_rstd,
                             void* dx, float* dgamma, float* dbeta, float* coef, float* workspace,
                             int B, int Di, int Hi, int Wi, int Do, int Ho, int Wo, int C, int relu, int accumulate, void* stream)
{
    hipStream_t st = (hipStream_t)stream;
    const int V = Di * Hi * Wi;
    if (C % 8 || B > BN_MAX_GRIDS) return DREG_EINVAL;
    const int rpc = bn_rows_per_chunk(V), nch = (V + rpc - 1) / rpc;
    const int CG = C / 8, slabs = (CG + 255) / 256;
    const dim3 grid(nch, B, slabs);
    hipLaunchKernelGGL((bn_pool_bwd_kernel<bf16_t, 0>), grid, dim3(256), 0, st, (const bf16_t*)x, (const bf16_t*)dp, argmax, mean_rstd, scale_shift, nullptr, workspace,
                       (bf16_t*)nullptr, Di, Hi, Wi, Do, Ho, Wo, C, rpc, relu);
    DREG_LAUNCH_CHECK();
    hipLaunchKernelGGL(bn_bwd_finalize_kernel, dim3(C), dim3(64 * (B < 8 ? B : 8)), 0, st, workspace, coef, dgamma, dbeta, B, nch, C, V, accumulate);
    DREG_LAUNCH_CHECK();
    hipLaunchKernelGGL((bn_pool_bwd_kernel<bf16_t, 1>), grid, dim3(256), 0, st, (const bf16_t*)x, (const bf16_t*)dp, argmax, mean_rstd, scale_shift, coef, nullptr,
                       (bf16_t*)dx, Di, Hi, Wi, Do, Ho, Wo, C, rpc, relu);
    DREG_LAUNCH_CHECK();
    return DREG_OK;
}
// ... 620 lines not shown
```

dreg_nerf_amd/lib.py:

```python
import ctypes
import os
from ctypes import c_float, c_int, c_size_t, c_void_p

import torch

_HERE = os.path.dirname(os.path.abspath(__file__))
LIB_PATH = os.path.join(_HERE, "libdreg_nerf_hip.so")

DT_BF16 = 0
DT_F32 = 1

_lib = None


class DregError(RuntimeError):
    pass


def _sig(lib, name, restype, argtypes):
    fn = getattr(lib, name)
    fn.restype = restype
    fn.argtypes = argtypes
    return fn

# ... 20 lines not shown
    "dreg_exec_guard_last": (I, [P, P, P, P]),
    "dreg_guard_fill": (I, [P, P, I, I, P]),
    "dreg_guard_scan": (I, [P, P, I, I, P, P]),
    "dreg_exec_create_opts": (P, [P, I, P, I, P, I, P]),
    "dreg_ps_set_group_wgrad": (None, [P, I]),
    "dreg_conv_get_glds": (I, []),
    "dreg_conv3d_dgrad_s2": (I, [P, P, P] + [I] * 11 + [P]),
    "dreg_conv3d_dgrad_s2_acc": (I, [P, P, P] + [I] * 11 + [P]),
    "dreg_pack_conv_weight": (I, [P, P, I, I, I, I, I, I, P]),
    "dreg_pack_conv_weights_batched": (I, [P, I, I, I, P, P]),
    "dreg_conv3d_wgrad_splits": (I, [I] * 8),
    "dreg_conv3d_wgrad_workspace_bytes": (Z, [I] * 8),
    "dreg_conv3d_wgrad": (I, [P, P, P, P, Z] + [I] * 16 + [P]),
    "dreg_conv3d_wgrad_occ": (I, [P, P, P, P, Z] + [I] * 16 + [P, P]),
    "dreg_conv3d_igemm_rows": (I, [P] * 5 + [P, I] + [I] * 18 + [I, P]),
    "dreg_conv3d_wgrad_rows": (I, [P, P, P, P, Z] + [P, I] + [I] * 14 + [P]),
    "dreg_conv3d_wgrad_partials": (I, [P, P, P, Z, P, I] + [I] * 13 + [P, P]),
    "dreg_wgrad_reduce_blocks": (I, [I, I, I, I]),
    "dreg_wgrad_reduce_batched": (I, [P, I, I, I, P]),
    "dreg_conv3_halo_supported": (I, [I] * 6),
    "dreg_conv3_halo_use": (I, [I] * 9),
    "dreg_conv3_halo_pack_bytes": (Z, [I]),
    "dreg_pack_conv_weight_halo": (I, [P, P, I, I, I, P]),
    "dreg_conv3_halo": (I, [P, P, P, P, P] + [I] * 10 + [P]),
    "dreg_conv3_halo_pack_bytes_n": (Z, [I, I]),
    "dreg_conv3_halo_n": (I, [P, P, P, P, P] + [I] * 11 + [P]),
    "dreg_conv3_halo_n_bnstats": (I, [P, P, P, P, P] + [I] * 10 + [P, P, P]),
    "dreg_conv1_stream_variant": (I, [I, I]),
    "dreg_conv1_stream_supported": (I, [I] * 14),
    "dreg_conv1_stream_use": (I, [I] * 14),
    "dreg_conv1_stream": (I, [P, P, P, P, P] + [I] * 20 + [P, Z, P, I]),
    "dreg_conv1_stream_bnstats": (I, [P, P, P, P, P] + [I] * 17 + [P, Z, P, P, P, I]),
    "dreg_conv3d_wgrad_variant": (I, [I] * 10),
    "dreg_conv3d_igemm_variant": (I, [I] * 17),
    "dreg_conv3d_wgrad_group_fill": (I, [P, P, P, P, Z] + [I] * 12 + [P, P]),
    "dreg_bn_small_in_regs": (I, [I, I, I, I]),
    "dreg_wgrad_group_desc_bytes": (I, []),
    "dreg_linear_wgrad_group_fill": (I, [P, P, P, P, Z, I, I, I, P, P]),
    "dreg_wgrad_group_launch": (I, [P, I, I, I, P]),
    "dreg_bn_num_chunks": (I, [I]),
    "dreg_bn_relu_maxpool_fwd": (I, [P] * 10 + [I] * 8 + [F, F, I, I, P]),
    "dreg_bn_relu_maxpool_bwd": (I, [P] * 10 + [I] * 10 + [P]),
    "dreg_sparse_stem_workspace_floats": (Z, [I] * 5),
    "dreg_sparse_stem_fwd": (I, [P, P, I, P, I] + [P] * 12 + [I] * 8 + [F, F, I, I, P]),
    "dreg_sparse_stem_bwd": (I, [P] * 6 + [I, P, I] + [P] * 7 + [I] * 10 + [P]),
    "dreg_bn3d_fwd": (I, [P] * 10 + [I, I, I, F, F, I, I, I, P]),
    "dreg_bn3d_bwd": (I, [P] * 11 + [I, I, I, I, I, I, P]),
    "dreg_bn_small": (I, [I, I, I, I]),
    "dreg_bn3d_fwd_defer_update": (I, [P] * 10 + [I, I, I, F, F, I, I, I, P, P, P]),
    "dreg_bn3d_fwd_from_sums": (I, [P] * 10 + [I, I, I, I, F, F, I, I, P]),
    "dreg_bn3d_bwd_defer_params": (I, [P] * 11 + [I, I, I, I, I, I, P, P, P]),
    "dreg_bn_running_update_batched": (I, [P, I, I, I, F, P]),
    "dreg_bn_param_grad_batched": (I, [P, I, I, I, I, P]),
    "dreg_maxpool3d_fwd": (I, [P, P, P] + [I] * 9 + [P]),
    "dreg_maxpool3d_bwd": (I, [P, P, P] + [I] * 9 + [P]),
    "dreg_maxpool3d_bwd_acc": (I, [P, P, P] + [I] * 10 + [P]),
    "dreg_downsample_sum": (I, [P, P] + [I] * 9 + [P]),
    "dreg_downsample_sum_rows": (I, [P, P, P] + [I] * 9 + [P]),
    "dreg_colsum_workspace_bytes": (Z, [Z, I]),
    "dreg_colsum": (I, [P, P, P, Z, I, I, I, P]),
    "dreg_trilinear_gather_fwd": (I, [P, P, P, P] + [I] * 10 + [P]),
    "dreg_trilinear_gather_bwd": (I, [P, P, P, P] + [I] * 8 + [P]),
    "dreg_cast_from_f32": (I, [P, P, Z, I, P]),
    "dreg_fill_zero": (I, [P, Z, P]),
    "dreg_active_sets_workspace_bytes": (Z, [I] * 4),
    "dreg_active_sets": (I, [P, P] + [I] * 8 + [P, P, P, P, Z, P]),
    "dreg_active_sets_level2_workspace_bytes": (Z, [I] * 4),
    "dreg_active_sets_level2": (I, [P] + [I] * 7 + [P, P, P, Z, P]),
    "dreg_conv_rows_workspace_bytes": (Z, [I, I, I, I]),
    "dreg_conv_rows": (I, [P, P, I, I, I, I, I, I, I, I, I, I, I, P, P, P, Z, P]),
    "dreg_trilinear_gather_bwd_rows": (I, [P, P, P, P, I, P, P, P] + [I] * 10 + [P]),
    "dreg_colsum_rows": (I, [P, P, I, P, P, I, I, I, P]),
    "dreg_trilinear_gather_bwd_gather": (I, [P, P, P, P, I, P, P] + [I] * 10 + [P]),
    "dreg_trilinear_gather_bwd_gather_rows_only": (I, [P, P, P, P, I, P, P] + [I] * 10 + [P]),
    "dreg_trilinear_gather_bwd_gather_seg": (I, [P, P, P, P, P, I, P, P] + [I] * 11 + [P]),
    "dreg_gather_segment_mean": (I, [P, P, P, I, P, P, P, P] + [I] * 9 + [P]),
    "dreg_zero_rows": (I, [P, P, I, I, I, P]),
    "dreg_add_inplace": (I, [P, P, Z, I, P]),
    "dreg_pack_rgba_grids": (I, [P, P, I, I, I, I, I, P]),
    "dreg_pack_rgba_grids_occ": (I, [P, P, P, I, I, I, I, I, P]),
    "dreg_pack_rgba_sparse": (I, [P, P, P, P, I, I, I, I, I, I, P]),
    "dreg_pack_rgba_sparse_occ": (I, [P, P, P, P, P, I, I, I, I, I, I, P]),
    "dreg_conv_row_occupancy": (I, [P, P, I, I, I, I, I, I, I, I, P]),
    "dreg_gather_grid_xyz": (I, [P, P, P, P, I, I, I, I, P]),
    "dreg_exec_create": (P, [P, I, P, I, P, I]),
    "dreg_exec_destroy": (None, [P]),
    "dreg_exec_op_halo": (I, [P, I]),
    "dreg_exec_op_pointwise": (I, [P, I]),
    "dreg_exec_op_wgrad_grouped": (I, [P, I]),
    "dreg_exec_arena_bytes": (Z, [P]),
    "dreg_exec_pack_bytes": (Z, [P]),
    "dreg_exec_num_packs": (I, [P]),
    "dreg_exec_tensor_offset": (Z, [P, I]),
    "dreg_exec_output_slot": (I, [P]),
    "dreg_exec_pack_rows": (I, [P]),
    "dreg_exec_export_pack_table": (I, [P, P, P, P]),
    "dreg_exec_repack": (I, [P, P, P, P]),
    "dreg_exec_set_overlap": (None, [P, I]),
    "dreg_exec_set_input_row_occupancy": (None, [P, P]),
    "dreg_exec_set_timing": (None, [P, I]),
    "dreg_exec_read_timings": (I, [P, P, P, I]),
    "dreg_exec_forward": (I, [P, P, Z, P, P, P, I, I, P]),
    "dreg_exec_backward": (I, [P, P, Z, P, P, P, P, I, P, P]),
    "dreg_exec_backward_range": (I, [P, P, Z, P, P, P, P, I, P, P, I, I, I]),
    "dreg_mha_fwd": (I, [P] * 5 + [I] * 7 + [F, I, P]),
    "dreg_mha_bwd": (I, [P] * 10 + [I] * 7 + [F, I, P]),
    "dreg_corr_attention_fwd": (I, [P] * 5 + [I] * 3 + [F, I, P]),
    "dreg_corr_attention_bwd": (I, [P] * 9 + [I] * 3 + [F, I, P]),
    "dreg_mha_varlen_fwd": (I, [P] * 6 + [I] * 9 + [F, I, P]),
    "dreg_mha_varlen_bwd": (I, [P] * 11 + [I] * 9 + [F, I, P]),
    "dreg_corr_attention_varlen_fwd": (I, [P] * 6 + [I] * 5 + [F, I, P]),
    "dreg_corr_attention_varlen_bwd": (I, [P] * 10 + [I] * 5 + [F, I, P]),
    "dreg_layernorm_fwd": (I, [P] * 6 + [I, I, F, I, P]),
    "dreg_layernorm_bwd_workspace_bytes": (Z, [I]),
    "dreg_layernorm_bwd": (I, [P] * 8 + [I] * 5 + [P]),
    "dreg_layernorm_bwd_add": (I, [P] * 9 + [I] * 4 + [P]),
    "dreg_layernorm_fwd2": (I, [P, P, P, P, I, P, P, P, I, I, F, P]),
    "dreg_layernorm_bwd_parts": (I, [P] * 10 + [I, I, I, P]),
    "dreg_layernorm_bwd_blocks": (I, [I]),
    "dreg_layernorm_bwd_final_batched": (I, [P, I, P]),
    "dreg_overlap_bwd_acc": (I, [P, P, P, P, P, P, P, P, I, P, I, P]),
    "dreg_colsum_rows_per_chunk": (I, [Z]),
    "dreg_colsum_batched": (I, [P, I, I, I, P]),
    "dreg_brick_supported": (I, [I] * 6),
    "dreg_conv3_brick_pack_bytes": (Z, [I, I]),
    "dreg_pack_conv_weight_brick": (I, [P, P, I, I, I, P]),
    "dreg_brick_tiles_workspace_bytes": (Z, [I] * 4),
    "dreg_brick_tiles_build": (I, [P, I, I, I, I, I, I, P, Z, P, P, P, P, P, P]),
    "dreg_conv3_brick": (I, [P, P, P, P, P, P, I, P, P, P] + [I] * 11 + [P]),
    "dreg_ps_num_params": (I, []),
    "dreg_ps_num_linears": (I, []),
    "dreg_ps_create": (P, [P]),
    "dreg_ps_destroy": (None, [P]),
    "dreg_ps_set_fuse": (None, [P, I]),
    "dreg_ps_set_timing": (None, [P, I]),
    "dreg_ps_read_timings": (I, [P, P, P, I]),
    "dreg_ps_arena_bytes": (Z, [P, I]),
    "dreg_ps_panel_fwd": (I, [P] * 13 + [I, I, I, I, F, P]),
    "dreg_ps_panel_bwd": (I, [P] * 12 + [I, I, I, P]),
    "dreg_ps_forward": (I, [P, P, Z, P, P, P, P, P, P, I, I, I, P, P, P, P]),
    "dreg_ps_backward": (I, [P, P, Z, P, P, P, P, P, P, I, I, I, P, P, P, P, P, P, P, P, P, I]),
# ... 60 lines not shown
    "dreg_ngp_render_train_samples": (I, [P, P, P, ctypes.c_long, P, I, I, I, P] + [P] * 6 + [P] * 5 + [P, P, P] + [F] * 5 + [P] + [P] * 5
                                      + [ctypes.c_long] + [P] * 9 + [P, P]),
    "dreg_ngp_samples_grad": (I, [ctypes.c_long] + [P] * 7 + [P] * 4 + [P] * 3 + [F] + [P] * 4),
    "dreg_ngp_points_input_grad": (I, [P, P, ctypes.c_long, P, P] + [P] * 5 + [P, P, P, P, P, P]),
    "dreg_ngp_samples_ray_grad": (I, [ctypes.c_long, P, P, P, P, ctypes.c_long, P, P, P]),
    "dreg_image_metrics_workspace_bytes": (Z, [I, I, I, I]),
    "dreg_image_metrics": (I, [P, P, I, I, I, I, P] + [P] * 6 + [P, Z, P]),
    "dreg_ngp_density_grad": (I, [P] * 7 + [P] * 5 + [P, I, I, P]),
    "dreg_icp_workspace_bytes": (Z, [I, I]),
    "dreg_icp_refine": (I, [P, I, P, P, P, P, I, P, F, I, I, I, P, F, I] + [ctypes.c_double] * 3 + [P, P, P, P, P, Z, P]),
    "dreg_icp_scene_workspace_bytes": (Z, [I, P, P]),
    "dreg_icp_scene_refine": (I, [I, P, P, P, F, I] + [ctypes.c_double] * 3 + [P, P, P, P, Z, P]),
    "dreg_pose_ransac_workspace_bytes": (Z, [I, I]),
    "dreg_pose_ransac": (I, [P, P, I, P, I, F, F, P, Z, P, P, P, P, P, P, P]),
    "dreg_pose_inliers": (I, [P, P, I, P, F, P, P, P]),
    "dreg_mc_table": (I, [P, P]),
    "dreg_mc_workspace_bytes": (Z, [I, I, I]),
    "dreg_mc_count": (I, [P, I, I, I, F, P, Z, P, P]),
    "dreg_mc_emit": (I, [P, I, I, I, F, P, P, P, Z, P, P, I, I, P]),
    "dreg_pair_density": (I, [P, ctypes.c_long, P, P, I, I, I] + ([P, I, I, I] + [P] * 3 + [P] * 5 + [P] * 3) * 2 + [P, F] + [P] * 5 + [P]),
    "dreg_scene_density": (I, [P, ctypes.c_long, P, P, I, I, I, I, P, F, P, P, P, P]),
    "dreg_scene_voxel_grid": (I, [I, I, I, P, P, I, P, F, F, F, P, P, P, P]),
}


PROBE_SIGNATURES = {
    "dreg_conv1_bnrelu_a_probe": (I, [P, P, P, P, I, I, I, I, I, I, P]),
    "dreg_conv_set_glds": (None, [I]),
    "dreg_conv_set_wgrad_splits": (None, [I]),
    "dreg_conv_set_wgrad_big": (None, [I]),
    "dreg_conv_igemm_probe": (None, [I]),
    "dreg_conv_set_igemm_ap": (None, [I]),
    "dreg_conv_set_igemm_ap256": (None, [I]),
    "dreg_conv_set_pointwise_rmw_cin": (None, [I]),
    "dreg_conv_igemm_probe_read": (I, [P]),
    "dreg_conv_set_wgrad_pipe": (None, [I]),
    "dreg_conv_wgrad_probe_read": (I, [P]),
    "dreg_conv_set_wgrad_ring": (None, [I]),
    "dreg_conv_set_wgrad_rows_fast": (None, [I]),
    "dreg_conv_set_row_splits": (None, [I]),
    "dreg_conv_set_glds_stages": (None, [I]),
    "dreg_conv_set_wgrad_target_blocks": (None, [I]),
    "dreg_conv_set_narrow_small": (None, [I]),
    "dreg_bn_set_debug_skip": (None, [I]),
    "dreg_bn_set_store_g": (None, [I]),
    "dreg_bn_set_small_regs": (None, [I]),
    "dreg_sstem_set_pool_blocks": (None, [I]),
    "dreg_voxel_set_own_sort": (None, [I]),
    "dreg_conv_set_bn_stats_epilogue": (None, [I]),
    "dreg_conv3_halo_set_variant": (None, [I]),
    "dreg_conv3_halo64_set": (None, [I]),
    "dreg_conv3_halo_set_prof": (None, [P]),
    "dreg_bn_set_small_max_voxels": (None, [I]),
    "dreg_ngp_set_rgb_chunks": (None, [I]),
    "dreg_ngp_set_density_unroll": (None, [I]),
    "dreg_ngp_set_xcd_levels": (None, [I]),
    "dreg_visibility_set_waves": (None, [I]),
    "dreg_visibility_set_pass_bound": (I, [ctypes.c_long]),
    "dreg_render_set_waves": (None, [I]),
    "dreg_render_pair_set_waves": (None, [I]),
    "dreg_render_bwd_set_waves": (None, [I]),
    "dreg_render_scene_set_waves": (None, [I]),
    "dreg_points_bwd_set_waves": (None, [I]),
    "dreg_render_samples_set_waves": (None, [I]),
    "dreg_scene_grid_set_waves": (None, [I]),
    "dreg_scene_grid_set_lanes_z": (None, [I]),
}
PROBE_LIB_PATH = os.path.join(_HERE, "libdreg_nerf_hip_probe.so")
_probe_lib = None


class ExecOpts(ctypes.Structure):
    _fields_ = [(n, c_int) for n in ("sparse_grads", "bn_batch_tails", "fuse_stem", "sparse_stem", "fold_res_bn", "fold_splitk", "group_wgrad",
                                     "s2_accumulate", "fuse_bn_stats", "brick", "defer_head_pg", "persistent_deep", "guard", "pointwise_stream")] + [("reserved", c_int * 2)]


SCENE_MAX_BLOCKS = 4


class SceneBlock(ctypes.Structure):
    _fields_ = ([("origins", P), ("viewdirs", P), ("binary", P), ("rx", c_int), ("ry", c_int), ("rz", c_int), ("coarse_bits", P)] +
                [(n, P) for n in ("table", "w1", "w2", "cw1", "cw2", "cw3", "offset", "size", "res", "scale", "hashed", "roi_aabb", "scene_aabb", "model_aabb")] +
                [(n, c_float) for n in ("near_plane", "far_plane", "render_step_size", "alpha_thre")] + [("center", P)])


class FieldBlock(ctypes.Structure):
    _fields_ = ([("binary", P), ("rx", c_int), ("ry", c_int), ("rz", c_int)] +
                [(n, P) for n in ("table", "w1", "w2", "offset", "size", "res", "scale", "hashed", "roi_aabb", "model_aabb", "center", "pose")])


class RadianceBlock(ctypes.Structure):
    _fields_ = [("field", FieldBlock)] + [(n, P) for n in ("cw1", "cw2", "cw3", "dirbias")]


class IcpBlock(ctypes.Structure):
    _fields_ = [("src", P), ("n", c_int), ("tgt_points", P), ("tgt_normals", P), ("cell_start", P), ("grid_lo", c_float * 3), ("cell", c_float),
                ("nx", c_int), ("ny", c_int), ("nz", c_int)]


def load_probe():
    global _probe_lib
    if _probe_lib is None:
        if not os.path.exists(PROBE_LIB_PATH):
            raise DregError(f"{PROBE_LIB_PATH} not found: build it with `python -m dreg_nerf_amd.build`")
        lib = ctypes.CDLL(PROBE_LIB_PATH)
        for name, (rt, at) in list(SIGNATURES.items()) + list(PROBE_SIGNATURES.items()):
            _sig(lib, name, rt, at)
        _probe_lib = lib
    return _probe_lib


def use_probe():
    global _lib
    _lib = load_probe()
    return _lib


class probe:

    def __init__(self):
        self._restore = []

    def __enter__(self):
        global _lib
        self._saved = _lib
        _lib = load_probe()
        self.lib = _lib
# ... 97 lines not shown
```

include/dreg_nerf.h:

```cpp
#ifndef DREG_NERF_H
#define DREG_NERF_H
#include <stddef.h>
#include <stdint.h>

#ifdef __cplusplus
extern "C" {
#endif

#define DREG_OK 0
#define DREG_EINVAL (-1)

int dreg_conv_get_glds(void);


int dreg_conv3d_kpad(int ksz, int Cin, int dtype);

int dreg_pack_conv_weight(const float* w, void* out, int Cout, int Cin_real, int Cin, int ksz, int for_dgrad,
                          int dtype, void* stream);
int dreg_pack_conv_weights_batched(const void* descs, int n, int total_rows, int stage_floats, const int* row_desc,
                                   void* stream);

int dreg_conv3d_igemm(const void* in, const void* wt_packed, void* out, const float* bias, const void* addend,
                      int B, int Di, int Hi, int Wi, int Cin, int Do, int Ho, int Wo, int Cout,
                      int ksz, int stride, int pad, int transposed, int relu, int Da, int Ha, int Wa, int add_same,
// ... 66 lines not shown
                           int ksz, int stride, int pad, int transposed, int relu, int Da, int Ha, int Wa, int add_same,
                           int out_f32, void* stream);
int dreg_conv3d_wgrad_rows(const void* gout, const void* in, float* dw, void* workspace, size_t workspace_bytes,
                           const int* rows, int nrows,
                           int B, int Di, int Hi, int Wi, int Cin, int Cin_real, int Do, int Ho, int Wo, int Cout,
                           int ksz, int stride, int pad, int accumulate, void* stream);
int dreg_conv3d_wgrad_partials(const void* gout, const void* in, void* workspace, size_t workspace_bytes, const int* rows, int nrows,
                               int B, int Di, int Hi, int Wi, int Cin, int Cin_real, int Do, int Ho, int Wo, int Cout,
                               int ksz, int stride, int pad, const uint8_t* rowocc, void* stream);
int dreg_wgrad_reduce_blocks(int Cout, int Cin_real, int ksz, int nsplit);
int dreg_wgrad_reduce_batched(const void* descs_dev, int n, int block_base, int nblocks, void* stream);
int dreg_wgrad_group_desc_bytes(void);
int dreg_linear_wgrad_group_fill(void* desc_host, const void* gout, const void* in, void* workspace, size_t workspace_bytes,
                                 int rows, int Cin, int Cout, int* variant, int* nblocks);
int dreg_conv3d_wgrad_group_fill(void* desc_host, const void* gout, const void* in, void* workspace, size_t workspace_bytes,
                                 int B, int Di, int Hi, int Wi, int Cin, int Do, int Ho, int Wo, int Cout, int ksz, int stride, int pad,
                                 int* variant, int* nblocks);
int dreg_wgrad_group_launch(const void* descs_dev, int n, int variant, int total_blocks, void* stream);

int dreg_bn_num_chunks(int V);
int dreg_bn3d_fwd(const void* x, const void* res, void* y, const float* gamma, const float* beta,
                  float* running_mean, float* running_var, float* scale_shift, float* mean_rstd, float* workspace,
                  int B, int V, int C, float eps, float momentum, int train, int relu, int dtype, void* stream);
int dreg_bn3d_bwd(const void* x, const void* dy, const void* y, const float* scale_shift, const float* mean_rstd,
                  void* dx, void* dres, float* dgamma, float* dbeta, float* coef, float* workspace,
                  int B, int V, int C, int relu, int accumulate, int dtype, void* stream);
int dreg_bn_small(int B, int V, int C, int dtype);
int dreg_bn3d_fwd_defer_update(const void* x, const void* res, void* y, const float* gamma, const float* beta,
                               float* running_mean, float* running_var, float* scale_shift, float* mean_rstd, float* workspace,
                               int B, int V, int C, float eps, float momentum, int train, int relu, int dtype, float* var_keep, int* deferred, void* stream);
int dreg_bn3d_bwd_defer_params(const void* x, const void* dy, const void* y, const float* scale_shift, const float* mean_rstd,
                               void* dx, void* dres, float* dgamma, float* dbeta, float* coef, float* workspace,
                               int B, int V, int C, int relu, int accumulate, int dtype, float* sums_keep, int* deferred, void* stream);
typedef struct dreg_bn_extra {
    const float* res_scale_shift;
    const float* splitk_part;
    int splitk_nsplit;
    size_t splitk_slice;
} dreg_bn_extra;
int dreg_bn3d_fwd_ex(const void* x, const void* res, void* y, const float* gamma, const float* beta,
                     float* running_mean, float* running_var, float* scale_shift, float* mean_rstd, float* workspace,
                     int B, int V, int C, float eps, float momentum, int train, int relu, int dtype, float* var_keep, int* deferred,
                     int sums_rows_per_chunk, const dreg_bn_extra* ex, void* stream);
int dreg_bn3d_bwd_ex(const void* x, const void* dy, const void* y, const float* scale_shift, const float* mean_rstd,
                     void* dx, void* dres, float* dgamma, float* dbeta, float* coef, float* workspace,
                     int B, int V, int C, int relu, int accumulate, int dtype, float* sums_keep, int* deferred, const dreg_bn_extra* ex, void* stream);
int dreg_conv3d_igemm_defer(const void* in, const void* wt_packed, void* out, const float* bias, const void* addend,
                            int B, int Di, int Hi, int Wi, int Cin, int Do, int Ho, int Wo, int Cout,
                            int ksz, int stride, int pad, int transposed, int relu, int Da, int Ha, int Wa, int add_same,
                            void* workspace, size_t workspace_bytes, const uint8_t* rowocc, int* sk_nsplit, size_t* sk_slice, void* stream);
int dreg_bn_small_in_regs(int B, int V, int C, int dtype);
int dreg_bn_running_update_batched(const void* descs_dev, int n, int block_base, int nblocks, float momentum, void* stream);
int dreg_bn_param_grad_batched(const void* descs_dev, int n, int block_base, int nblocks, int accumulate, void* stream);

int dreg_bn_relu_maxpool_fwd(const void* x, void* pooled, uint8_t* argmax, const float* gamma, const float* beta,
                             float* running_mean, float* running_var, float* scale_shift, float* mean_rstd, float* workspace,
                             int B, int Di, int Hi, int Wi, int Do, int Ho, int Wo, int C, float eps, float momentum, int train, int relu, void* stream);
int dreg_bn_relu_maxpool_bwd(const void* x, const void* dp, const uint8_t* argmax, const float* scale_shift, const float* mean_rstd,
                             void* dx, float* dgamma, float* dbeta, float* coef, float* workspace,
                             int B, int Di, int Hi, int Wi, int Do, int Ho, int Wo, int C, int relu, int accumulate, void* stream);
size_t dreg_sparse_stem_workspace_floats(int B, int Do, int Ho, int Wo, int C);
int dreg_sparse_stem_fwd(const void* x, const int* rows, int n, const int* rows_a, int n_a, void* act, void* pooled, uint8_t* argmax, void* xam, uint8_t* pmask,
                         const float* gamma, const float* beta, float* running_mean, float* running_var, float* scale_shift, float* mean_rstd, float* workspace,
                         int B, int Di, int Hi, int Wi, int Do, int Ho, int Wo, int C, float eps, float momentum, int train, int relu, void* stream);
int dreg_sparse_stem_bwd(const void* x, const void* dp, const uint8_t* argmax, const void* xam, const void* dl, const int* rows_a, int n_a,
                         const int* rows, int n, const float* scale_shift, const float* mean_rstd, void* dx, float* dgamma, float* dbeta, float* coef, float* workspace,
                         int B, int Di, int Hi, int Wi, int Do, int Ho, int Wo, int C, int relu, int accumulate, void* stream);
int dreg_maxpool3d_fwd(const void* x, void* y, uint8_t* argmax, int B, int Di, int Hi, int Wi, int Do, int Ho, int Wo,
                       int C, int dtype, void* stream);
int dreg_maxpool3d_bwd(const void* dy, const uint8_t* argmax, void* dx, int B, int Di, int Hi, int Wi, int Do, int Ho,
                       int Wo, int C, int dtype, void* stream);
int dreg_maxpool3d_bwd_acc(const void* dy, const uint8_t* argmax, void* dx, int B, int Di, int Hi, int Wi, int Do, int Ho,
                           int Wo, int C, int accumulate, int dtype, void* stream);

int dreg_downsample_sum(const void* g, void* out, int B, int Df, int Hf, int Wf, int Dc, int Hc, int Wc, int C,
                        int dtype, void* stream);
int dreg_downsample_sum_rows(const void* g, void* out, const int* rows, int nrows, int Df, int Hf, int Wf, int Dc, int Hc, int Wc,
                             int C, int dtype, void* stream);

size_t dreg_colsum_workspace_bytes(size_t M, int C);
int dreg_colsum(const void* g, float* out, float* workspace, size_t M, int C, int accumulate, int dtype, void* stream);

int dreg_trilinear_gather_fwd(const void* p1, const int64_t* idx, const int* pt_batch, void* out, int N, int d, int h,
                              int w, int C, int Zr, int Xr, int Yr, int dtype, int out_f32, void* stream);
int dreg_trilinear_gather_bwd(const float* dfeat, const int64_t* idx, const int* pt_batch, float* dp1_f32, int N, int d,
                              int h, int w, int C, int Zr, int Xr, int Yr, void* stream);
int dreg_cast_from_f32(const float* in, void* out, size_t n, int dtype, void* stream);
int dreg_fill_zero(void* p, size_t bytes, void* stream);
int dreg_guard_fill(void* base, const void* offsets_dev, int n, int band_bytes, void* stream);
int dreg_guard_scan(const void* base, const void* offsets_dev, int n, int band_bytes, void* result_dev, void* stream);
int dreg_colsum_rows_per_chunk(size_t M);
int dreg_colsum_batched(const void* descs_dev, int n, int total_pblocks, int total_fblocks, void* stream);
int dreg_add_inplace(void* dst, const void* src, size_t n, int dtype, void* stream);
int dreg_pack_rgba_grids(const void* grids, void* out, int B, int Z, int X, int Y, int dtype, void* stream);
int dreg_pack_rgba_grids_occ(const void* grids, void* out, uint8_t* inocc, int B, int Z, int X, int Y, int dtype, void* stream);
int dreg_pack_rgba_sparse(const float* vals, const int64_t* idx, const int* pt_batch, void* out, int N, int B, int Z, int X,
                          int Y, int dtype, void* stream);
int dreg_pack_rgba_sparse_occ(const float* vals, const int64_t* idx, const int* pt_batch, void* out, uint8_t* inocc, int N, int B, int Z, int X,
                              int Y, int dtype, void* stream);
int dreg_conv_row_occupancy(const uint8_t* inocc, uint8_t* rowocc, int B, int Di, int Hi, int Do, int Ho, int ksz, int stride, int pad, void* stream);
int dreg_gather_grid_xyz(const void* grids, const int64_t* idx, const int* pt_batch, float* xyz, int N, int Zr, int Xr, int Yr,
                         void* stream);

size_t dreg_active_sets_workspace_bytes(int B, int d, int h, int w);
int dreg_active_sets(const int64_t* idx, const int* pt_batch, int N, int B, int Zr, int Xr, int Yr, int d, int h, int w,
                     int* rows, int* counts, int* map1, void* workspace, size_t workspace_bytes, void* stream);
size_t dreg_active_sets_level2_workspace_bytes(int B, int d2, int h2, int w2);
int dreg_active_sets_level2(const uint8_t* child_flags, int B, int d, int h, int w, int d2, int h2, int w2, int* rows2,
                            int* counts2, void* workspace, size_t workspace_bytes, void* stream);
size_t dreg_conv_rows_workspace_bytes(int B, int d, int h, int w);
int dreg_conv_rows(const int64_t* idx, const int* pt_batch, int N, int B, int Zr, int Xr, int Yr, int d, int h, int w, int ksz, int stride, int pad,
                   int* rows, int* count, void* workspace, size_t workspace_bytes, void* stream);
int dreg_trilinear_gather_bwd_rows(const float* dfeat, const int64_t* idx, const int* pt_batch, const int* rows1, int n1,
                                   const int* map1, float* comp, void* dp1, int N, int B, int d, int h, int w, int C,
                                   int Zr, int Xr, int Yr, int dtype, void* stream);
int dreg_trilinear_gather_bwd_gather(const float* dfeat, const int64_t* idx, const int* pt_batch, const int* rows1, int n1,
                                     int* fine_map, void* dp1, int N, int B, int d, int h, int w, int C, int Zr, int Xr,
                                     int Yr, int dtype, void* stream);
int dreg_trilinear_gather_bwd_gather_rows_only(const float* dfeat, const int64_t* idx, const int* pt_batch, const int* rows1, int n1,
                                               int* fine_map, void* dp1, int N, int B, int d, int h, int w, int C, int Zr, int Xr, int Yr,
                                               int dtype, void* stream);
int dreg_trilinear_gather_bwd_gather_seg(const float* g1, const void* seg_descs, const int64_t* idx, const int* pt_batch, const int* rows1, int n1,
                                         int* fine_map, void* dp1, int N, int B, int d, int h, int w, int C, int Zr, int Xr, int Yr,
                                         int dtype, int zero_dense, void* stream);
int dreg_gather_segment_mean(const void* p1, const int64_t* idx, const int* pt_batch, int point_start, const uint32_t* order, const uint32_t* starts,
                             const int* n_out, float* out, int M, int d, int h, int w, int C, int Zr, int Xr, int Yr, int dtype, void* stream);
int dreg_zero_rows(void* buf, const int* rows, int nrows, int C, int dtype, void* stream);
int dreg_colsum_rows(const void* g, const int* rows, int nrows, float* out, float* workspace, int C, int accumulate,
                     int dtype, void* stream);

void* dreg_exec_create(const int* tensors, int nt, const int* ops, int nops, const int64_t* params, int np);
typedef struct dreg_exec_opts {
    int sparse_grads;
    int bn_batch_tails;
    int fuse_stem;
    int sparse_stem;
    int fold_res_bn;
    int fold_splitk;
    int group_wgrad;
    int s2_accumulate;
    int fuse_bn_stats;
    int brick;
    int defer_head_pg;
    int persistent_deep;
    int guard;
    int pointwise_stream;
    int reserved[2];
} dreg_exec_opts;
void dreg_exec_default_opts(dreg_exec_opts* o);
void* dreg_exec_create_opts(const int* tensors, int nt, const int* ops, int nops, const int64_t* params, int np, const dreg_exec_opts* opts);
#define DREG_EGUARD (-3)
int dreg_exec_guard_bands(void* h);
int dreg_exec_guard_check(void* h, void* arena, long long* out4, void* stream);
int dreg_exec_guard_describe(void* h, int band, char* buf, int buf_bytes);
int dreg_exec_guard_last(void* h, int* op, int* pass, long long* band);
void dreg_exec_destroy(void* h);
size_t dreg_exec_arena_bytes(void* h);
size_t dreg_exec_pack_bytes(void* h);
int dreg_exec_num_packs(void* h);
size_t dreg_exec_tensor_offset(void* h, int slot);
int dreg_exec_output_slot(void* h);
int dreg_exec_pack_rows(void* h);
int dreg_exec_export_pack_table(void* h, void* host_out, int* host_row_desc, void* pack_base);
int dreg_exec_repack(void* h, const void* descs_dev, const int* row_desc_dev, void* stream);
int dreg_exec_op_halo(void* h, int op);
int dreg_exec_op_wgrad_grouped(void* h, int op);
int dreg_exec_op_pointwise(void* h, int op);
void dreg_exec_set_overlap(void* h, int enable);
void dreg_exec_set_input_row_occupancy(void* h, const uint8_t* rowocc);
void dreg_exec_set_timing(void* h, int enable);
int dreg_exec_read_timings(void* h, int* op_kind, float* ms, int max);
int dreg_exec_forward(void* h, void* arena, size_t arena_bytes, const void* pack_base, const void* x_in,
                      const int64_t* rowlists, int nlists, int train, void* stream);
int dreg_exec_backward(void* h, void* arena, size_t arena_bytes, const void* pack_base, const void* x_in,
                       const void* grad_out, const int64_t* rowlists, int nlists, void* stream, void* aux_stream);
int dreg_exec_backward_range(void* h, void* arena, size_t arena_bytes, const void* pack_base, const void* x_in, const void* grad_out,
                             const int64_t* rowlists, int nlists, void* stream, void* aux_stream, int op_begin, int op_end, int flags);

int dreg_mha_fwd(const void* q, const void* k, const void* v, void* o, float* lse, int Nq, int Nk, int H,
                 int ldq, int ldk, int ldv, int ldo, float scale, int dtype, void* stream);
int dreg_mha_bwd(const void* q, const void* k, const void* v, const void* o, const void* dout, const float* lse,
                 float* dvec, void* dq, void* dk, void* dv, int Nq, int Nk, int H,
                 int ldq, int ldk, int ldv, int ldo, float scale, int dtype, void* stream);
int dreg_corr_attention_fwd(const void* q, const void* k, const float* xyz, float* out, float* lse, int L, int Nq, int Nk,
                            float scale, int dtype, void* stream);
int dreg_corr_attention_bwd(const void* q, const void* k, const float* xyz, const float* out, const float* dout,
                            const float* lse, float* dvec, void* dq, void* dk, int L, int Nq, int Nk,
                            float scale, int dtype, void* stream);

int dreg_mha_varlen_fwd(const void* q, const void* k, const void* v, void* o, float* lse, const int* probs, int nprob,
                        int max_q, int max_k, int R, int H, int ldq, int ldk, int ldv, int ldo, float scale, int dtype, void* stream);
int dreg_mha_varlen_bwd(const void* q, const void* k, const void* v, const void* o, const void* dout, const float* lse,
                        float* dvec, void* dq, void* dk, void* dv, const int* probs, int nprob, int max_q, int max_k, int R, int H,
                        int ldq, int ldk, int ldv, int ldo, float scale, int dtype, void* stream);
int dreg_corr_attention_varlen_fwd(const void* q, const void* k, const float* xyz, float* out, float* lse, const int* probs, int nprob,
                                   int max_q, int max_k, int L, int R, float scale, int dtype, void* stream);
int dreg_corr_attention_varlen_bwd(const void* q, const void* k, const float* xyz, const float* out, const float* dout,
                                   const float* lse, float* dvec, void* dq, void* dk, const int* probs, int nprob,
                                   int max_q, int max_k, int L, int R, float scale, int dtype, void* stream);

int dreg_layernorm_fwd(const float* x, const float* gamma, const float* beta, const float* pe, void* y, float* stats,
                       int N, int C, float eps, int out_dtype, void* stream);
size_t dreg_layernorm_bwd_workspace_bytes(int N);
int dreg_layernorm_bwd(const float* x, const void* dy, const float* gamma, const float* stats, float* dx, float* dgamma,
                       float* dbeta, float* workspace, int N, int C, int g_dtype, int accumulate_dx, int accumulate_w,
                       void* stream);
int dreg_layernorm_bwd_add(const float* x, const void* dy, const float* gamma, const float* stats, float* dx, const float* dx_add, float* dgamma,
                           float* dbeta, float* workspace, int N, int C, int g_dtype, int accumulate_w, void* stream);

int dreg_layernorm_fwd2(const float* x, const float* gamma, const float* beta, const float* pe, int pe_rows, float* y32, void* y16, float* stats,
                        int N, int C, float eps, void* stream);
int dreg_layernorm_bwd_parts(const float* x, const void* dy, const void* dy2_bf16, const float* gamma, const float* stats, float* dx, const float* dx_add,
                             const float* dx_add2, void* dx_bf16, float* part, int N, int C, int g_dtype, void* stream);
int dreg_layernorm_bwd_blocks(int N);
int dreg_layernorm_bwd_final_batched(const void* descs_dev, int n, void* stream);

int dreg_posenc_sine(const float* xyz, float* pe, int N, float scale, float temperature, void* stream);

int dreg_overlap_fwd(const float* f, const float* w, const float* b, float* s, int N, void* stream);
// ... 306 lines not shown
```

include/dreg_nerf_probe.h:

```cpp
#ifndef DREG_NERF_PROBE_H
#define DREG_NERF_PROBE_H
#ifdef __cplusplus
extern "C" {
#endif

void dreg_conv3_halo_set_variant(int variant);
void dreg_conv3_halo64_set(int v);
void dreg_conv3_halo_set_prof(void* u64_buf_64x8x5);
void dreg_conv_set_glds(int enable);
int dreg_conv1_bnrelu_a_probe(const void* in, const void* wt_packed, void* out, const float* a_scale_shift, int B, int D, int H, int W, int Cin, int Cout, void* stream);
void dreg_conv_set_wgrad_splits(int splits);
void dreg_conv_set_wgrad_rows_fast(int enable);
void dreg_conv_set_row_splits(int on);
void dreg_conv_set_wgrad_ring(int mode);
int dreg_conv_wgrad_probe_read(unsigned long long* out8);
void dreg_conv_set_wgrad_pipe(int enable);
void dreg_conv_set_igemm_ap(int max_tiles);
void dreg_conv_set_pointwise_rmw_cin(int max_cin);
void dreg_conv_set_igemm_ap256(int on);
void dreg_conv_igemm_probe(int enable);
int dreg_conv_igemm_probe_read(unsigned long long* out6);
void dreg_conv_set_wgrad_big(int mode);
void dreg_conv_set_glds_stages(int stages);
void dreg_conv_set_wgrad_target_blocks(int blocks);
void dreg_bn_set_small_max_voxels(int v);
void dreg_sstem_set_pool_blocks(int n);
void dreg_voxel_set_own_sort(int on);
void dreg_conv_set_bn_stats_epilogue(int on);
void dreg_bn_set_store_g(int enable);
void dreg_bn_set_small_regs(int enable);
void dreg_bn_set_debug_skip(int mask);
void dreg_ngp_set_rgb_chunks(int on);
void dreg_ngp_set_density_unroll(int n);
void dreg_ngp_set_xcd_levels(int on);
int dreg_visibility_set_pass_bound(long passes);
void dreg_visibility_set_waves(int n);
void dreg_render_set_waves(int n);
void dreg_render_pair_set_waves(int n);
void dreg_render_scene_set_waves(int n);
void dreg_render_bwd_set_waves(int n);
void dreg_points_bwd_set_waves(int n);
void dreg_render_samples_set_waves(int n);
void dreg_conv_set_narrow_small(int on);
void dreg_scene_grid_set_waves(int n);
void dreg_scene_grid_set_lanes_z(int on);

#ifdef __cplusplus
}
#endif
#endif
```

Baseline: 263.4 pairs/s.

## Let BN apply kernels compute their own coefficients from partial sums

Adds a self-coefficient BatchNorm path for mid-sized layers. The forward and backward apply kernels reduce the per-chunk partial sums themselves, which removes the separate finalize kernel launches between the stats pass and the apply pass. Running-stat and parameter-gradient updates go to the batched tail kernels through double-precision keep buffers. The cost is redundant reduction work in every apply block and more arena space, and the executor now has extra branching for which BN path each op takes.

```diff
diff --git a/dreg_nerf_amd/csrc/executor.hip b/dreg_nerf_amd/csrc/executor.hip
--- a/dreg_nerf_amd/csrc/executor.hip
+++ b/dreg_nerf_amd/csrc/executor.hip
@@ -52,6 +52,7 @@
     int fold_into = -1, res_from = -1;
     int bt = -1;
     size_t keep_var = 0, keep_sums = 0;
+    int self_coef = 0;
 };
 struct HaloPack { const float* w; size_t off; int Cout, Cin, transposed, brick; };
 struct PackRec { const float* w; void* out; int Cout, Cin_real, inner, ntaps, for_dgrad, Kpad, dtype, row0; };
@@ -157,6 +158,7 @@
     std::memset(o, 0, sizeof(*o));
     o->sparse_grads = 1; o->bn_batch_tails = 1; o->fuse_stem = 1; o->sparse_stem = 1; o->fold_res_bn = 1; o->fold_splitk = 1;
     o->group_wgrad = 1; o->s2_accumulate = 1; o->fuse_bn_stats = 1; o->brick = 1; o->defer_head_pg = 0; o->pointwise_stream = 1;
+    o->bn_self_coef = 1;
 }
 void* dreg_exec_create(const int* tensors, int nt, const int* ops, int nops, const int64_t* params, int np)
 {
@@ -169,7 +171,7 @@
     e->opt.brick &= 3;
     const int g_sparse_grads = e->opt.sparse_grads, g_bn_batch_tails = e->opt.bn_batch_tails, g_fuse_stem = e->opt.fuse_stem, g_sparse_stem = e->opt.sparse_stem,
               g_fold_res_bn = e->opt.fold_res_bn, g_fold_splitk = e->opt.fold_splitk, g_group_wgrad = e->opt.group_wgrad, g_fuse_bn_stats = e->opt.fuse_bn_stats,
-              g_brick = e->opt.brick;
+              g_brick = e->opt.brick, g_bn_self_coef = e->opt.bn_self_coef;
     e->t.resize(nt);
     for (int i = 0; i < nt; ++i) {
         Tensor& t = e->t[i];
@@ -286,6 +288,19 @@
                 BnTailRec f{}, b{};
                 f.a = (const float*)o.aux1; f.b = (const float*)o.keep_var; f.o0 = e->prm[o.p2].val; f.o1 = e->prm[o.p3].val;
                 b.a = (const float*)o.keep_sums; b.b = nullptr; b.o0 = e->prm[o.w].grad; b.o1 = e->prm[o.b].grad;
+                f.B = b.B = x.B; f.V = b.V = (int)V; f.C = b.C = x.C; f.block0 = b.block0 = e->bn_blocks;
+                e->bn_blocks += (x.C + 255) / 256;
+                o.bt = (int)e->bn_fwd.size();
+                e->bn_fwd.push_back(f); e->bn_bwd.push_back(b);
+            } else if (g_bn_self_coef && g_bn_batch_tails && o.pool < 0 && !shared && o.fold_into < 0 &&
+                       (dreg_bn_self_coef_use(x.B, (int)V, x.C, 0, 0) || dreg_bn_self_coef_use(x.B, (int)V, x.C, 0, 1))) {
+                o.self_coef = (dreg_bn_self_coef_use(x.B, (int)V, x.C, 0, 0) ? 1 : 0) | (dreg_bn_self_coef_use(x.B, (int)V, x.C, 0, 1) ? 2 : 0);
+                const size_t kb = align256((size_t)x.B * x.C * 2 * sizeof(double));
+                o.keep_var = off; off += kb;
+                o.keep_sums = off; off += kb;
+                BnTailRec f{}, b{};
+                f.b = (const float*)o.keep_var; f.o0 = e->prm[o.p2].val; f.o1 = e->prm[o.p3].val;
+                b.b = (const float*)o.keep_sums; b.o0 = e->prm[o.w].grad; b.o1 = e->prm[o.b].grad;
                 f.B = b.B = x.B; f.V = b.V = (int)V; f.C = b.C = x.C; f.block0 = b.block0 = e->bn_blocks;
                 e->bn_blocks += (x.C + 255) / 256;
                 o.bt = (int)e->bn_fwd.size();
@@ -520,6 +535,7 @@
 }
 int dreg_exec_op_halo(void* h, int op) { Exec* e = (Exec*)h; return op >= 0 && op < (int)e->ops.size() ? e->ops[op].halo : 0; }
 int dreg_exec_op_wgrad_grouped(void* h, int op) { Exec* e = (Exec*)h; return op >= 0 && op < (int)e->ops.size() ? e->ops[op].grp : 0; }
+int dreg_exec_op_bn_self_coef(void* h, int op) { Exec* e = (Exec*)h; return op >= 0 && op < (int)e->ops.size() ? e->ops[op].self_coef : 0; }
 int dreg_exec_op_pointwise(void* h, int op) { Exec* e = (Exec*)h; return op >= 0 && op < (int)e->ops.size() ? e->ops[op].pointwise : 0; }
 
 void dreg_exec_set_overlap(void* h, int enable) { ((Exec*)h)->use_aux = enable != 0; }
@@ -575,8 +591,12 @@
     e->reduce_abs = e->reduce;
     for (ReduceRec& r : e->reduce_abs) r.part = (const float*)(A + (size_t)r.part);
     std::vector<BnTailRec> f = e->bn_fwd, b = e->bn_bwd;
-    for (BnTailRec& r : f) { r.a = (const float*)(A + (size_t)r.a); r.b = (const float*)(A + (size_t)r.b); }
-    for (BnTailRec& r : b) r.a = (const float*)(A + (size_t)r.a);
+    for (size_t q = 0; q < f.size(); ++q) {
+        const bool self = e->bn_fwd[q].a == nullptr && e->bn_bwd[q].b != nullptr;
+        f[q].b = (const float*)(A + (size_t)f[q].b);
+        if (self) b[q].b = (const float*)(A + (size_t)b[q].b);
+        else { f[q].a = (const float*)(A + (size_t)f[q].a); b[q].a = (const float*)(A + (size_t)b[q].a); }
+    }
     if (!e->reduce_abs.empty() && hipMemcpyAsync(A + e->off_rd, e->reduce_abs.data(), e->reduce_abs.size() * sizeof(ReduceRec), hipMemcpyHostToDevice, st) != hipSuccess) return DREG_ELAUNCH;
     if (!f.empty() && (hipMemcpyAsync(A + e->off_bnf, f.data(), f.size() * sizeof(BnTailRec), hipMemcpyHostToDevice, st) != hipSuccess ||
                        hipMemcpyAsync(A + e->off_bnb, b.data(), b.size() * sizeof(BnTailRec), hipMemcpyHostToDevice, st) != hipSuccess)) return DREG_ELAUNCH;
@@ -757,6 +777,12 @@
             void* out_p = o.fold_into >= 0 ? nullptr : act(o.out);
             dreg_bn_extra ex{};
             if (o.res_from >= 0) { res_p = act(e->ops[o.res_from].in); ex.res_scale_shift = (const float*)(A + e->ops[o.res_from].aux0); }
+            if (train && sums_rpc[i] > 0 && (o.self_coef & 1) && out_p) {
+                CK(dreg_bn3d_fwd_self_coef(act(o.in), res_p, out_p, e->prm[o.w].val, e->prm[o.b].val, (float*)(A + o.aux0), (float*)(A + o.aux1),
+                                           (float*)(A + o.stats_off), sums_rpc[i], x.B, V, x.C, 1e-5f, o.relu, 0, (double*)(A + o.keep_var), ex.res_scale_shift, stream));
+                bn_done[o.bt] = 1;
+                continue;
+            }
             if (train && sums_rpc[i] > 0) {
                 CK(dreg_bn3d_fwd_ex(act(o.in), res_p, out_p, e->prm[o.w].val, e->prm[o.b].val, e->prm[o.p2].val, e->prm[o.p3].val,
                                     (float*)(A + o.aux0), (float*)(A + o.aux1), (float*)(A + o.stats_off), x.B, V, x.C, 1e-5f, 0.1f, 1, o.relu, 0,
@@ -767,7 +793,7 @@
             if (fwd_sk_bn == (int)i) { ex.splitk_part = (const float*)(A + e->off_ks); ex.splitk_nsplit = fwd_sk_n; ex.splitk_slice = fwd_sk_slice; fwd_sk_bn = -1; }
             CK(dreg_bn3d_fwd_ex(act(o.in), res_p, out_p, e->prm[o.w].val, e->prm[o.b].val, e->prm[o.p2].val, e->prm[o.p3].val,
                                 (float*)(A + o.aux0), (float*)(A + o.aux1), (float*)(A + e->off_bn_ws), x.B, V, x.C, 1e-5f, 0.1f, train, o.relu, 0,
-                                o.bt >= 0 ? (float*)(A + o.keep_var) : nullptr, &deferred, 0, &ex, stream));
+                                o.bt >= 0 && !o.self_coef ? (float*)(A + o.keep_var) : nullptr, &deferred, 0, &ex, stream));
             if (deferred) bn_done[o.bt] = 1;
         } else if (o.kind == OP_MAXPOOL) {
             CK(dreg_maxpool3d_fwd(act(o.in), act(o.out), (uint8_t*)(A + o.aux0), x.B, x.D, x.H, x.W, y.D, y.H, y.W, x.C, 0, stream));
@@ -1090,18 +1116,26 @@
             if (res_via_copy) {
                 CK(dreg_bn3d_bwd_defer_params(act(o.in), gy, act(o.out), (float*)(A + o.aux0), (float*)(A + o.aux1), dx, nullptr, e->prm[o.w].grad, e->prm[o.b].grad,
                                               (float*)(A + e->off_coef), (float*)(A + e->off_bn_ws), x.B, V, x.C, o.relu, 1, 0,
-                                              o.bt >= 0 ? (float*)(A + o.keep_sums) : nullptr, &deferred, stream));
+                                              o.bt >= 0 && !o.self_coef ? (float*)(A + o.keep_sums) : nullptr, &deferred, stream));
                 if (deferred) bn_done[o.bt] = 1;
                 CK(commit(o.in));
                 if (o.relu) CK(dreg_relu_bwd(act(o.out), gy, A + e->off_tmp, (size_t)x.B * V * x.C, 0, 0, 0, stream));
                 else if (hipMemcpyAsync(A + e->off_tmp, gy, (size_t)x.B * V * x.C * 2, hipMemcpyDeviceToDevice, st) != hipSuccess) return DREG_ELAUNCH;
                 CK(commit(o.in2));
             } else {
+                if ((o.self_coef & 2) && e->pend_sk_bn != i) {
+                    CK(dreg_bn3d_bwd_self_coef(act(o.in), gy, o.in2 >= 0 ? act(o.out) : nullptr, (float*)(A + o.aux0), (float*)(A + o.aux1), dx, dres,
+                                               (float*)(A + e->off_bn_ws), x.B, V, x.C, o.relu, 0, (double*)(A + o.keep_sums), stream));
+                    bn_done[o.bt] = 1;
+                    if (res_g && dres == (void*)(A + e->off_tmp)) { CK(commit(o.in2)); CK(commit(o.in)); }
+                    else { CK(commit(o.in)); if (res_g) CK(commit(o.in2)); }
+                    continue;
+                }
                 dreg_bn_extra ex{};
                 if (e->pend_sk_bn == i) { ex.splitk_part = (const float*)(A + e->off_ks); ex.splitk_nsplit = e->pend_sk_n; ex.splitk_slice = e->pend_sk_slice; e->pend_sk_bn = -1; }
                 CK(dreg_bn3d_bwd_ex(act(o.in), gy, o.in2 >= 0 ? act(o.out) : nullptr, (float*)(A + o.aux0), (float*)(A + o.aux1), dx, dres, e->prm[o.w].grad, e->prm[o.b].grad,
                                     (float*)(A + e->off_coef), (float*)(A + e->off_bn_ws), x.B, V, x.C, o.relu, 1, 0,
-                                    o.bt >= 0 ? (float*)(A + o.keep_sums) : nullptr, &deferred, &ex, stream));
+                                    o.bt >= 0 && !o.self_coef ? (float*)(A + o.keep_sums) : nullptr, &deferred, &ex, stream));
                 if (deferred) bn_done[o.bt] = 1;
                 if (res_g && dres == (void*)(A + e->off_tmp)) { CK(commit(o.in2)); CK(commit(o.in)); }
                 else { CK(commit(o.in)); if (res_g) CK(commit(o.in2)); }
diff --git a/dreg_nerf_amd/csrc/fpn_ops.hip b/dreg_nerf_amd/csrc/fpn_ops.hip
--- a/dreg_nerf_amd/csrc/fpn_ops.hip
+++ b/dreg_nerf_amd/csrc/fpn_ops.hip
@@ -139,6 +139,70 @@
     }
 }
 
+__device__ __forceinline__ const float* bn_chunk_ptr(const float* __restrict__ partial, int b, int k, int c, int nchunks, int C)
+{
+    return partial + (((size_t)b * nchunks + k) * C + c) * 2;
+}
+__device__ __forceinline__ void bn_chunk_sums_wave(const float* __restrict__ partial, int b, int c, int nchunks, int C, int lane, double& s1, double& s2)
+{
+    s1 = 0.0; s2 = 0.0;
+#pragma unroll 8
+    for (int k = lane; k < nchunks; k += 64) {
+        const float2 p = *reinterpret_cast<const float2*>(bn_chunk_ptr(partial, b, k, c, nchunks, C));
+        s1 += p.x; s2 += p.y;
+    }
+    s1 = wave_sum_d(s1); s2 = wave_sum_d(s2);
+}
+constexpr int BNSC_P = 4, BNSC_M = 64 / BNSC_P, BNSC_CH = 256 / BNSC_P;
+static_assert(BNSC_P == 4, "bn_chunk_sums_join is written for four threads per channel");
+__device__ __forceinline__ void bn_chunk_sums_part(const float* __restrict__ partial, int b, int c, int nchunks, int C, int j, double& s1, double& s2)
+{
+    double a1[BNSC_M], a2[BNSC_M];
+#pragma unroll
+    for (int m = 0; m < BNSC_M; ++m) a1[m] = a2[m] = 0.0;
+    for (int k0 = 0; k0 < nchunks; k0 += 64) {
+#pragma unroll
+        for (int m = 0; m < BNSC_M; ++m) {
+            const int k = k0 + j + BNSC_P * m;
+            const bool ok = k < nchunks;
+            const float2 p = *reinterpret_cast<const float2*>(bn_chunk_ptr(partial, b, ok ? k : 0, c, nchunks, C));
+            a1[m] += ok ? (double)p.x : 0.0; a2[m] += ok ? (double)p.y : 0.0;
+        }
+    }
+#pragma unroll
+    for (int h = BNSC_M / 2; h > 0; h >>= 1)
+#pragma unroll
+        for (int m = 0; m < h; ++m) { a1[m] += a1[m + h]; a2[m] += a2[m + h]; }
+    s1 = a1[0]; s2 = a2[0];
+}
+__device__ __forceinline__ double bn_chunk_sums_join(double t0, double t1, double t2, double t3) { return (t0 + t2) + (t1 + t3); }
+
+struct BnFwdCoef { double mean, var; float scale, shift, rstd; };
+__device__ __forceinline__ BnFwdCoef bn_fwd_coef(double s1, double s2, int V, float ga, float be, float eps)
+{
+    BnFwdCoef k;
+    const double mean = s1 / V;
+    double var = s2 / V - mean * mean;
+    if (var < 0) var = 0;
+    const float rstd = 1.0f / sqrtf((float)var + eps);
+    k.mean = mean; k.var = var; k.rstd = rstd;
+    k.scale = ga * rstd;
+    k.shift = be - (float)mean * ga * rstd;
+    return k;
+}
+__device__ __forceinline__ void bn_fwd_coef_store(const BnFwdCoef& k, float* __restrict__ scale_shift, float* __restrict__ mean_rstd, size_t pc)
+{
+    scale_shift[pc] = k.scale; scale_shift[pc + 1] = k.shift;
+    mean_rstd[pc] = (float)k.mean; mean_rstd[pc + 1] = k.rstd;
+}
+__device__ __forceinline__ void bn_running_step(float& rm, float& rv, double mean, double var, int V, float momentum)
+{
+    const float unbiased = V > 1 ? (float)(var * V / (V - 1)) : (float)var;
+    rm = (1.f - momentum) * rm + momentum * (float)mean;
+    rv = (1.f - momentum) * rv + momentum * unbiased;
+}
+__device__ __forceinline__ void bn_bwd_coef(double s1, double s2, int V, float& c1, float& c2) { c1 = (float)(s1 / V); c2 = (float)(s2 / V); }
+
 constexpr int BN_MAX_GRIDS = 256;
 __global__ __launch_bounds__(512) void bn_finalize_kernel(const float* __restrict__ partial, const float* __restrict__ gamma, const float* __restrict__ beta,
                                    float* __restrict__ running_mean, float* __restrict__ running_var,
@@ -159,34 +223,18 @@
     }
     __shared__ double stat[BN_MAX_GRIDS][2];
     for (int b = wave; b < B; b += nw) {
-        double s1 = 0.0, s2 = 0.0;
-#pragma unroll 8
-        for (int k = lane; k < nchunks; k += 64) {
-            const float2 p = *reinterpret_cast<const float2*>(partial + (((size_t)b * nchunks + k) * C + c) * 2);
-            s1 += p.x; s2 += p.y;
-        }
-        s1 = wave_sum_d(s1); s2 = wave_sum_d(s2);
-        const double mean = s1 / V;
-        double var = s2 / V - mean * mean;
-        if (var < 0) var = 0;
+        double s1, s2;
+        bn_chunk_sums_wave(partial, b, c, nchunks, C, lane, s1, s2);
+        const BnFwdCoef k = bn_fwd_coef(s1, s2, V, ga, be, eps);
         if (lane == 0) {
-            const float rstd = 1.0f / sqrtf((float)var + eps);
-            scale_shift[((size_t)b * C + c) * 2] = ga * rstd;
-            scale_shift[((size_t)b * C + c) * 2 + 1] = be - (float)mean * ga * rstd;
-            mean_rstd[((size_t)b * C + c) * 2] = (float)mean;
-            mean_rstd[((size_t)b * C + c) * 2 + 1] = rstd;
-            stat[b][0] = mean; stat[b][1] = var;
+            bn_fwd_coef_store(k, scale_shift, mean_rstd, ((size_t)b * C + c) * 2);
+            stat[b][0] = k.mean; stat[b][1] = k.var;
         }
     }
     __syncthreads();
     if (threadIdx.x == 0) {
         float rm = running_mean[c], rv = running_var[c];
-        for (int b = 0; b < B; ++b) {
-            const double mean = stat[b][0], var = stat[b][1];
-            const float unbiased = V > 1 ? (float)(var * V / (V - 1)) : (float)var;
-            rm = (1.f - momentum) * rm + momentum * (float)mean;
-            rv = (1.f - momentum) * rv + momentum * unbiased;
-        }
+        for (int b = 0; b < B; ++b) bn_running_step(rm, rv, stat[b][0], stat[b][1], V, momentum);
         running_mean[c] = rm; running_var[c] = rv;
     }
 }
@@ -220,16 +268,10 @@
     const int c = blockIdx.x, wave = threadIdx.x >> 6, lane = threadIdx.x & 63, nw = blockDim.x >> 6;
     __shared__ double stat[BN_MAX_GRIDS][2];
     for (int b = wave; b < B; b += nw) {
-        double s1 = 0.0, s2 = 0.0;
-#pragma unroll 8
-        for (int k = lane; k < nchunks; k += 64) {
-            const float2 p = *reinterpret_cast<const float2*>(partial + (((size_t)b * nchunks + k) * C + c) * 2);
-            s1 += p.x; s2 += p.y;
-        }
-        s1 = wave_sum_d(s1); s2 = wave_sum_d(s2);
+        double s1, s2;
+        bn_chunk_sums_wave(partial, b, c, nchunks, C, lane, s1, s2);
         if (lane == 0) {
-            coef[((size_t)b * C + c) * 2] = (float)(s1 / V);
-            coef[((size_t)b * C + c) * 2 + 1] = (float)(s2 / V);
+            bn_bwd_coef(s1, s2, V, coef[((size_t)b * C + c) * 2], coef[((size_t)b * C + c) * 2 + 1]);
             stat[b][0] = s1; stat[b][1] = s2;
         }
     }
@@ -274,21 +316,11 @@
 }
 
 template <typename T, int UN>
-__global__ __launch_bounds__(256) void bn_apply_cols_kernel(const T* __restrict__ x, const float* __restrict__ scale_shift, const T* __restrict__ res,
-                                                            T* __restrict__ y, int V, int C, int rows_per_chunk, int relu,
-                                                            const float* __restrict__ res_ss = nullptr)
+__device__ __forceinline__ void bn_apply_cols_walk(const T* __restrict__ x, const T* __restrict__ res, T* __restrict__ y, int b, int cg, int r0, int rpi,
+                                                   int v0, int v1, int V, int C, int relu, bool res_ss,
+                                                   const float (&sc)[Gran<T>::G], const float (&sh)[Gran<T>::G], const float (&rsc)[Gran<T>::G], const float (&rsh)[Gran<T>::G])
 {
     constexpr int G = Gran<T>::G;
-    const int CG = C / G, cgs = CG < 256 ? CG : 256, rpi = 256 / cgs;
-    const int t = threadIdx.x, cg = blockIdx.z * cgs + (t % cgs), r0 = t / cgs, b = blockIdx.y;
-    if (r0 >= rpi || cg >= CG) return;
-    const int v0 = blockIdx.x * rows_per_chunk, v1 = min(v0 + rows_per_chunk, V);
-    float sc[G], sh[G], rsc[G], rsh[G];
-#pragma unroll
-    for (int i = 0; i < G; ++i) {
-        sc[i] = scale_shift[((size_t)b * C + cg * G + i) * 2]; sh[i] = scale_shift[((size_t)b * C + cg * G + i) * 2 + 1];
-        if (res_ss) { rsc[i] = res_ss[((size_t)b * C + cg * G + i) * 2]; rsh[i] = res_ss[((size_t)b * C + cg * G + i) * 2 + 1]; }
-    }
     for (int v = v0 + r0; v < v1; v += rpi * UN) {
         float xv[UN][G], rv[UN][G];
 #pragma unroll
@@ -316,6 +348,63 @@
     }
 }
 template <typename T, int UN>
+__global__ __launch_bounds__(256) void bn_apply_cols_kernel(const T* __restrict__ x, const float* __restrict__ scale_shift, const T* __restrict__ res,
+                                                            T* __restrict__ y, int V, int C, int rows_per_chunk, int relu,
+                                                            const float* __restrict__ res_ss = nullptr)
+{
+    constexpr int G = Gran<T>::G;
+    const int CG = C / G, cgs = CG < 256 ? CG : 256, rpi = 256 / cgs;
+    const int t = threadIdx.x, cg = blockIdx.z * cgs + (t % cgs), r0 = t / cgs, b = blockIdx.y;
+    if (r0 >= rpi || cg >= CG) return;
+    const int v0 = blockIdx.x * rows_per_chunk, v1 = min(v0 + rows_per_chunk, V);
+    float sc[G], sh[G], rsc[G], rsh[G];
+#pragma unroll
+    for (int i = 0; i < G; ++i) {
+        sc[i] = scale_shift[((size_t)b * C + cg * G + i) * 2]; sh[i] = scale_shift[((size_t)b * C + cg * G + i) * 2 + 1];
+        if (res_ss) { rsc[i] = res_ss[((size_t)b * C + cg * G + i) * 2]; rsh[i] = res_ss[((size_t)b * C + cg * G + i) * 2 + 1]; }
+    }
+    bn_apply_cols_walk<T, UN>(x, res, y, b, cg, r0, rpi, v0, v1, V, C, relu, res_ss != nullptr, sc, sh, rsc, rsh);
+}
+template <typename T, int UN>
+__device__ __forceinline__ void bn_bwd_apply_cols_walk(const T* __restrict__ x, const T* dy, const T* __restrict__ y, T* __restrict__ dx, T* dres, int b, int cg, int r0, int rpi,
+                                                       int v0, int v1, int V, int C, int relu,
+                                                       const float (&mu)[Gran<T>::G], const float (&rs)[Gran<T>::G], const float (&sc)[Gran<T>::G], const float (&sh)[Gran<T>::G],
+                                                       const float (&c1)[Gran<T>::G], const float (&c2)[Gran<T>::G])
+{
+    constexpr int G = Gran<T>::G;
+    const bool remask = relu && y == nullptr;
+    for (int v = v0 + r0; v < v1; v += rpi * UN) {
+        float xv[UN][G], gv[UN][G], yv[UN][G];
+#pragma unroll
+        for (int u = 0; u < UN; ++u)
+            if (v + u * rpi < v1) {
+                const size_t off = ((size_t)b * V + v + u * rpi) * C + (size_t)cg * G;
+                Gran<T>::ld(x + off, xv[u]);
+                Gran<T>::ld(dy + off, gv[u]);
+                if (relu && !remask) Gran<T>::ld(y + off, yv[u]);
+            }
+#pragma unroll
+        for (int u = 0; u < UN; ++u)
+            if (v + u * rpi < v1) {
+                const size_t off = ((size_t)b * V + v + u * rpi) * C + (size_t)cg * G;
+                if (remask) {
+#pragma unroll
+                    for (int k = 0; k < G; ++k) gv[u][k] = (xv[u][k] * sc[k] + sh[k]) > 0.f ? gv[u][k] : 0.f;
+                } else if (relu) {
+#pragma unroll
+                    for (int k = 0; k < G; ++k) gv[u][k] = yv[u][k] > 0.f ? gv[u][k] : 0.f;
+                }
+                if (dres) Gran<T>::st(dres + off, gv[u]);
+#pragma unroll
+                for (int k = 0; k < G; ++k) {
+                    const float xh = (xv[u][k] - mu[k]) * rs[k];
+                    xv[u][k] = sc[k] * (gv[u][k] - c1[k] - xh * c2[k]);
+                }
+                Gran<T>::st(dx + off, xv[u]);
+            }
+    }
+}
+template <typename T, int UN>
 __global__ __launch_bounds__(256) void bn_bwd_apply_cols_kernel(const T* __restrict__ x, const T* dy, const T* __restrict__ y,
                                                                 const float* __restrict__ mean_rstd, const float* __restrict__ scale_shift,
                                                                 const float* __restrict__ coef, T* __restrict__ dx, T* dres,
@@ -333,37 +422,89 @@
         const size_t pc = ((size_t)b * C + cg * G + i) * 2;
         mu[i] = mean_rstd[pc]; rs[i] = mean_rstd[pc + 1]; sc[i] = scale_shift[pc]; sh[i] = scale_shift[pc + 1]; c1[i] = coef[pc]; c2[i] = coef[pc + 1];
     }
-    const bool remask = relu && y == nullptr;
-    for (int v = v0 + r0; v < v1; v += rpi * UN) {
-        float xv[UN][G], gv[UN][G], yv[UN][G];
-#pragma unroll
-        for (int u = 0; u < UN; ++u)
-            if (v + u * rpi < v1) {
-                const size_t off = ((size_t)b * V + v + u * rpi) * C + (size_t)cg * G;
-                Gran<T>::ld(x + off, xv[u]);
-                Gran<T>::ld(dy + off, gv[u]);
-                if (relu && !remask) Gran<T>::ld(y + off, yv[u]);
+    bn_bwd_apply_cols_walk<T, UN>(x, dy, y, dx, dres, b, cg, r0, rpi, v0, v1, V, C, relu, mu, rs, sc, sh, c1, c2);
+}
+
+constexpr int BNSC_MAXC = 128;
+template <int PASS>
+__device__ __forceinline__ void bn_self_prologue(const float* __restrict__ sums, int b, int c_lo, int nc, int nchunks, int C, int V,
+                                                 const float* __restrict__ gamma, const float* __restrict__ beta, float eps,
+                                                 float* __restrict__ scale_shift, float* __restrict__ mean_rstd, double* __restrict__ keep, bool writer,
+                                                 float (*s_out)[BNSC_MAXC], double (*red)[BNSC_CH][2])
+{
+    const int ci = threadIdx.x % BNSC_CH, j = threadIdx.x / BNSC_CH;
+    for (int cr = 0; cr < nc; cr += BNSC_CH) {
+        const bool valid = cr + ci < nc;
+        const int c = c_lo + cr + ci;
+        double s1 = 0.0, s2 = 0.0;
+        if (valid) {
+            bn_chunk_sums_part(sums, b, c, nchunks, C, j, s1, s2);
+            red[j][ci][0] = s1; red[j][ci][1] = s2;
+        }
+        __syncthreads();
+        if (valid && j == 0) {
+            s1 = bn_chunk_sums_join(s1, red[1][ci][0], red[2][ci][0], red[3][ci][0]);
+            s2 = bn_chunk_sums_join(s2, red[1][ci][1], red[2][ci][1], red[3][ci][1]);
+            const size_t pc = ((size_t)b * C + c) * 2;
+            if (PASS == 0) {
+                const BnFwdCoef k = bn_fwd_coef(s1, s2, V, gamma[c], beta[c], eps);
+                s_out[0][cr + ci] = k.scale; s_out[1][cr + ci] = k.shift;
+                if (writer) { bn_fwd_coef_store(k, scale_shift, mean_rstd, pc); keep[pc] = k.mean; keep[pc + 1] = k.var; }
+            } else {
+                bn_bwd_coef(s1, s2, V, s_out[0][cr + ci], s_out[1][cr + ci]);
+                if (writer) { keep[pc] = s1; keep[pc + 1] = s2; }
             }
-#pragma unroll
-        for (int u = 0; u < UN; ++u)
-            if (v + u * rpi < v1) {
-                const size_t off = ((size_t)b * V + v + u * rpi) * C + (size_t)cg * G;
-                if (remask) {
-#pragma unroll
-                    for (int k = 0; k < G; ++k) gv[u][k] = (xv[u][k] * sc[k] + sh[k]) > 0.f ? gv[u][k] : 0.f;
-                } else if (relu) {
-#pragma unroll
-                    for (int k = 0; k < G; ++k) gv[u][k] = yv[u][k] > 0.f ? gv[u][k] : 0.f;
-                }
-                if (dres) Gran<T>::st(dres + off, gv[u]);
-#pragma unroll
-                for (int k = 0; k < G; ++k) {
-                    const float xh = (xv[u][k] - mu[k]) * rs[k];
-                    xv[u][k] = sc[k] * (gv[u][k] - c1[k] - xh * c2[k]);
-                }
-                Gran<T>::st(dx + off, xv[u]);
-            }
-    }
+        }
+        __syncthreads();
+    }
+}
+template <typename T, int UN>
+__global__ __launch_bounds__(256) void bn_apply_self_kernel(const T* __restrict__ x, const float* __restrict__ sums, const float* __restrict__ gamma,
+                                                            const float* __restrict__ beta, const T* __restrict__ res, T* __restrict__ y,
+                                                            float* __restrict__ scale_shift, float* __restrict__ mean_rstd, double* __restrict__ keep,
+                                                            int V, int C, int nchunks, int rows_per_wg, float eps, int relu, const float* __restrict__ res_ss)
+{
+    constexpr int G = Gran<T>::G, CGS = BNSC_MAXC / G;
+    const int CG = C / G, cgs = CG < CGS ? CG : CGS, rpi = 256 / cgs;
+    const int t = threadIdx.x, lg = t % cgs, cg = blockIdx.z * cgs + lg, r0 = t / cgs, b = blockIdx.y;
+    __shared__ float s_out[2][BNSC_MAXC];
+    __shared__ double red[BNSC_P][BNSC_CH][2];
+    const int c_lo = blockIdx.z * cgs * G;
+    bn_self_prologue<0>(sums, b, c_lo, min(cgs * G, C - c_lo), nchunks, C, V, gamma, beta, eps, scale_shift, mean_rstd, keep, blockIdx.x == 0, s_out, red);
+    if (r0 >= rpi || cg >= CG) return;
+    const int v0 = blockIdx.x * rows_per_wg, v1 = min(v0 + rows_per_wg, V);
+    float sc[G], sh[G], rsc[G], rsh[G];
+#pragma unroll
+    for (int i = 0; i < G; ++i) {
+        sc[i] = s_out[0][lg * G + i]; sh[i] = s_out[1][lg * G + i];
+        if (res_ss) { rsc[i] = res_ss[((size_t)b * C + cg * G + i) * 2]; rsh[i] = res_ss[((size_t)b * C + cg * G + i) * 2 + 1]; }
+    }
+    bn_apply_cols_walk<T, UN>(x, res, y, b, cg, r0, rpi, v0, v1, V, C, relu, res_ss != nullptr, sc, sh, rsc, rsh);
+}
+template <typename T, int UN>
+__global__ __launch_bounds__(256) void bn_bwd_apply_self_kernel(const T* __restrict__ x, const T* dy, const T* __restrict__ y, const float* __restrict__ sums,
+                                                                const float* __restrict__ mean_rstd, const float* __restrict__ scale_shift,
+                                                                T* __restrict__ dx, T* dres, double* __restrict__ keep,
+                                                                int V, int C, int nchunks, int rows_per_wg, int relu, int g_stored)
+{
+    constexpr int G = Gran<T>::G, CGS = BNSC_MAXC / G;
+    const int CG = C / G, cgs = CG < CGS ? CG : CGS, rpi = 256 / cgs;
+    const int t = threadIdx.x, lg = t % cgs, cg = blockIdx.z * cgs + lg, r0 = t / cgs, b = blockIdx.y;
+    __shared__ float s_out[2][BNSC_MAXC];
+    __shared__ double red[BNSC_P][BNSC_CH][2];
+    const int c_lo = blockIdx.z * cgs * G;
+    bn_self_prologue<1>(sums, b, c_lo, min(cgs * G, C - c_lo), nchunks, C, V, nullptr, nullptr, 0.f, nullptr, nullptr, keep, blockIdx.x == 0, s_out, red);
+    if (r0 >= rpi || cg >= CG) return;
+    if (g_stored) { dy = dres; dres = nullptr; relu = 0; }
+    const int v0 = blockIdx.x * rows_per_wg, v1 = min(v0 + rows_per_wg, V);
+    float mu[G], rs[G], sc[G], sh[G], c1[G], c2[G];
+#pragma unroll
+    for (int i = 0; i < G; ++i) {
+        const size_t pc = ((size_t)b * C + cg * G + i) * 2;
+        mu[i] = mean_rstd[pc]; rs[i] = mean_rstd[pc + 1]; sc[i] = scale_shift[pc]; sh[i] = scale_shift[pc + 1];
+        c1[i] = s_out[0][lg * G + i]; c2[i] = s_out[1][lg * G + i];
+    }
+    bn_bwd_apply_cols_walk<T, UN>(x, dy, y, dx, dres, b, cg, r0, rpi, v0, v1, V, C, relu, mu, rs, sc, sh, c1, c2);
 }
 
 constexpr int BNS_COLS = 4, BNS_ROWS = 64;
@@ -650,6 +791,20 @@
     const BnTailDesc d = descs[lo];
     const int c = (blk - d.block0) * blockDim.x + threadIdx.x;
     if (c >= d.C) return;
+    if (d.a == nullptr) {
+        const double* p = reinterpret_cast<const double*>(d.b);
+        if (WHAT == 0) {
+            float rm = d.o0[c], rv = d.o1[c];
+            for (int b = 0; b < d.B; ++b) bn_running_step(rm, rv, p[((size_t)b * d.C + c) * 2], p[((size_t)b * d.C + c) * 2 + 1], d.V, momentum);
+            d.o0[c] = rm; d.o1[c] = rv;
+        } else {
+            double dg = 0.0, db = 0.0;
+            for (int b = 0; b < d.B; ++b) { db += p[((size_t)b * d.C + c) * 2]; dg += p[((size_t)b * d.C + c) * 2 + 1]; }
+            d.o0[c] = accumulate ? d.o0[c] + (float)dg : (float)dg;
+            d.o1[c] = accumulate ? d.o1[c] + (float)db : (float)db;
+        }
+        return;
+    }
     if (WHAT == 0) {
         float rm = d.o0[c], rv = d.o1[c];
         for (int b = 0; b < d.B; ++b) {
@@ -1772,6 +1927,15 @@
     return (int)(b > (size_t)cap ? cap : (b ? b : 1));
 }
 static inline bool slabs_ragged(int CG) { return CG > 256 && CG % 256 != 0; }
+DREG_KNOB(int, g_bn_self_wgs, 512);
+static inline int bn_rows_per_chunk(int V);
+static inline int bn_self_slabs(int C, int G) { const int CG = C / G, cgs = CG < BNSC_MAXC / G ? CG : BNSC_MAXC / G; return (CG + cgs - 1) / cgs; }
+static inline int bn_self_rows(int B, int V, int C, int G)
+{
+    int rows = bn_rows_per_chunk(V);
+    while (rows < V && (long long)((V + rows - 1) / rows) * B * bn_self_slabs(C, G) > g_bn_self_wgs) rows *= 2;
+    return rows;
+}
 static inline int bn_rows_per_chunk(int V) { return V >= 262144 ? 512 : V >= 32768 ? 256 : V >= 4096 ? 128 : V >= 512 ? 32 : (V >= 8 ? 8 : V); }
 
 extern "C" {
@@ -1781,13 +1945,14 @@
 void dreg_bn_set_store_g(int enable) { g_bn_store_g = enable ? 1 : 0; }
 void dreg_bn_set_small_regs(int enable) { g_bn_small_regs = enable ? 1 : 0; }
 void dreg_bn_set_small_max_voxels(int v) { g_bn_small_maxv = v; }
+void dreg_bn_set_self_wgs(int n) { g_bn_self_wgs = n > 0 ? n : 512; }
 #endif
 int dreg_bn_num_chunks(int V) { const int r = bn_rows_per_chunk(V); return (V + r - 1) / r; }
 
 static int bn3d_fwd_impl(const void* x, const void* res, void* y, const float* gamma, const float* beta,
                          float* running_mean, float* running_var, float* scale_shift, float* mean_rstd, float* workspace,
                          int B, int V, int C, float eps, float momentum, int train, int relu, int dtype, void* stream, float* var_keep, int* deferred,
-                         int sums_rows_per_chunk = 0, const dreg_bn_extra* ex = nullptr);
+                         int sums_rows_per_chunk = 0, const dreg_bn_extra* ex = nullptr, double* self_keep = nullptr);
 int dreg_bn3d_fwd(const void* x, const void* res, void* y, const float* gamma, const float* beta,
                   float* running_mean, float* running_var, float* scale_shift, float* mean_rstd, float* workspace,
                   int B, int V, int C, float eps, float momentum, int train, int relu, int dtype, void* stream)
@@ -1818,19 +1983,29 @@
                          sums_rows_per_chunk > 0 ? 1 : train, relu, dtype, stream, var_keep, deferred, sums_rows_per_chunk, ex);
 }
 int dreg_bn_small(int B, int V, int C, int dtype) { return bn_small_ok(B, V, C, dtype == 0 ? 8 : 4) ? 1 : 0; }
-int dreg_bn_running_update_batched(const void* descs_dev, int n, int block_base, int nblocks, float momentum, void* stream)
-{
-    if (n <= 0 || nblocks <= 0) return DREG_OK;
-    hipLaunchKernelGGL(bn_tail_batched_kernel<0>, dim3(nblocks), dim3(256), 0, (hipStream_t)stream, (const BnTailDesc*)descs_dev, n, block_base, momentum, 0);
-    DREG_LAUNCH_CHECK();
-    return DREG_OK;
-}
-int dreg_bn_param_grad_batched(const void* descs_dev, int n, int block_base, int nblocks, int accumulate, void* stream)
-{
-    if (n <= 0 || nblocks <= 0) return DREG_OK;
-    hipLaunchKernelGGL(bn_tail_batched_kernel<1>, dim3(nblocks), dim3(256), 0, (hipStream_t)stream, (const BnTailDesc*)descs_dev, n, block_base, 0.f, accumulate);
-    DREG_LAUNCH_CHECK();
-    return DREG_OK;
+int dreg_bn_self_coef_supported(int B, int V, int C, int dtype)
+{
+    const int G = dtype == 0 ? 8 : 4;
+    return (B >= 1 && B <= BN_MAX_GRIDS && V >= 2 && C >= G && C % G == 0 && !slabs_ragged(C / G) && !bn_small_ok(B, V, C, G)) ? 1 : 0;
+}
+int dreg_bn_self_coef_use(int B, int V, int C, int dtype, int backward)
+{
+    if (!dreg_bn_self_coef_supported(B, V, C, dtype) || dtype != 0 || B < 2 || B > 16) return 0;
+    if (V == 4096) return (C == 128 || C == 256 || C == 512) ? 1 : 0;
+    if (V == 32768) return (backward && (C == 64 || C == 256)) ? 1 : 0;
+    return 0;
+}
+int dreg_bn_self_coef_rows(int B, int V, int C, int dtype) { return bn_self_rows(B, V, C, dtype == 0 ? 8 : 4); }
+int dreg_bn3d_fwd_self_coef(const void* x, const void* res, void* y, const float* gamma, const float* beta, float* scale_shift, float* mean_rstd,
+                            float* sums, int rows_per_chunk, int B, int V, int C, float eps, int relu, int dtype, double* keep,
+                            const float* res_scale_shift, void* stream)
+{
+    if (rows_per_chunk <= 0 || !keep) return DREG_EINVAL;
+    dreg_bn_extra ex{};
+    ex.res_scale_shift = res_scale_shift;
+    int deferred = 0;
+    return bn3d_fwd_impl(x, res, y, gamma, beta, nullptr, nullptr, scale_shift, mean_rstd, sums, B, V, C, eps, 0.f, 1, relu, dtype, stream, nullptr, &deferred,
+                         rows_per_chunk, &ex, keep);
 }
 struct BnSplitkIn { const float* part = nullptr; int nsplit = 0; size_t slice = 0; };
 int dreg_bn_small_in_regs(int B, int V, int C, int dtype)
@@ -1840,7 +2015,7 @@
 static int bn3d_fwd_impl(const void* x, const void* res, void* y, const float* gamma, const float* beta,
                          float* running_mean, float* running_var, float* scale_shift, float* mean_rstd, float* workspace,
                          int B, int V, int C, float eps, float momentum, int train, int relu, int dtype, void* stream, float* var_keep, int* deferred,
-                         int sums_rows_per_chunk, const dreg_bn_extra* ex)
+                         int sums_rows_per_chunk, const dreg_bn_extra* ex, double* self_keep)
 {
     hipStream_t st = (hipStream_t)stream;
     const float* res_ss = ex ? ex->res_scale_shift : nullptr;
@@ -1871,6 +2046,18 @@
         return DREG_OK;
     }
     if (train && V < 2) return DREG_EINVAL;
+    if (self_keep) {
+        if (!presummed || !y || !deferred || !dreg_bn_self_coef_supported(B, V, C, dtype)) return DREG_EINVAL;
+        const int rows = bn_self_rows(B, V, C, G);
+        const dim3 sgrid((V + rows - 1) / rows, B, bn_self_slabs(C, G));
+        if (dtype == 0) hipLaunchKernelGGL((bn_apply_self_kernel<bf16_t, 4>), sgrid, dim3(256), 0, st, (const bf16_t*)x, workspace, gamma, beta, (const bf16_t*)res, (bf16_t*)y, scale_shift, mean_rstd, self_keep,
+                                           V, C, V / sums_rows_per_chunk, rows, eps, relu, res ? res_ss : nullptr);
+        else hipLaunchKernelGGL((bn_apply_self_kernel<float, 4>), sgrid, dim3(256), 0, st, (const float*)x, workspace, gamma, beta, (const float*)res, (float*)y, scale_shift, mean_rstd, self_keep,
+                                V, C, V / sums_rows_per_chunk, rows, eps, relu, res ? res_ss : nullptr);
+        DREG_LAUNCH_CHECK();
+        *deferred = 1;
+        return DREG_OK;
+    }
     if (B > BN_MAX_GRIDS || (train && !presummed && slabs_ragged(CG))) return DREG_EINVAL;
     if (train && !presummed && !(g_bn_debug_skip & 1)) {
         dim3 grid(nch, B, slabs);
@@ -1891,7 +2078,7 @@
 
 static int bn3d_bwd_impl(const void* x, const void* dy, const void* y, const float* scale_shift, const float* mean_rstd,
                          void* dx, void* dres, float* dgamma, float* dbeta, float* coef, float* workspace,
-                         int B, int V, int C, int relu, int accumulate, int dtype, void* stream, float* sums_keep, int* deferred, const dreg_bn_extra* ex = nullptr);
+                         int B, int V, int C, int relu, int accumulate, int dtype, void* stream, float* sums_keep, int* deferred, const dreg_bn_extra* ex = nullptr, double* self_keep = nullptr);
 int dreg_bn3d_bwd(const void* x, const void* dy, const void* y, const float* scale_shift, const float* mean_rstd,
                   void* dx, void* dres, float* dgamma, float* dbeta, float* coef, float* workspace,
                   int B, int V, int C, int relu, int accumulate, int dtype, void* stream)
@@ -1910,9 +2097,30 @@
 {
     return bn3d_bwd_impl(x, dy, y, scale_shift, mean_rstd, dx, dres, dgamma, dbeta, coef, workspace, B, V, C, relu, accumulate, dtype, stream, sums_keep, deferred, ex);
 }
+int dreg_bn3d_bwd_self_coef(const void* x, const void* dy, const void* y, const float* scale_shift, const float* mean_rstd,
+                            void* dx, void* dres, float* workspace, int B, int V, int C, int relu, int dtype, double* keep, void* stream)
+{
+    if (!keep) return DREG_EINVAL;
+    int deferred = 0;
+    return bn3d_bwd_impl(x, dy, y, scale_shift, mean_rstd, dx, dres, nullptr, nullptr, nullptr, workspace, B, V, C, relu, 0, dtype, stream, nullptr, &deferred, nullptr, keep);
+}
+int dreg_bn_running_update_batched(const void* descs_dev, int n, int block_base, int nblocks, float momentum, void* stream)
+{
+    if (n <= 0 || nblocks <= 0) return DREG_OK;
+    hipLaunchKernelGGL(bn_tail_batched_kernel<0>, dim3(nblocks), dim3(256), 0, (hipStream_t)stream, (const BnTailDesc*)descs_dev, n, block_base, momentum, 0);
+    DREG_LAUNCH_CHECK();
+    return DREG_OK;
+}
+int dreg_bn_param_grad_batched(const void* descs_dev, int n, int block_base, int nblocks, int accumulate, void* stream)
+{
+    if (n <= 0 || nblocks <= 0) return DREG_OK;
+    hipLaunchKernelGGL(bn_tail_batched_kernel<1>, dim3(nblocks), dim3(256), 0, (hipStream_t)stream, (const BnTailDesc*)descs_dev, n, block_base, 0.f, accumulate);
+    DREG_LAUNCH_CHECK();
+    return DREG_OK;
+}
 static int bn3d_bwd_impl(const void* x, const void* dy, const void* y, const float* scale_shift, const float* mean_rstd,
                          void* dx, void* dres, float* dgamma, float* dbeta, float* coef, float* workspace,
-                         int B, int V, int C, int relu, int accumulate, int dtype, void* stream, float* sums_keep, int* deferred, const dreg_bn_extra* ex)
+                         int B, int V, int C, int relu, int accumulate, int dtype, void* stream, float* sums_keep, int* deferred, const dreg_bn_extra* ex, double* self_keep)
 {
     hipStream_t st = (hipStream_t)stream;
     BnSplitkIn ski;
@@ -1924,6 +2132,7 @@
     const int rpc = bn_rows_per_chunk(V), nch = (V + rpc - 1) / rpc;
     const int CG = C / G, slabs = (CG + 255) / 256;
     if (bn_small_ok(B, V, C, G)) {
+        if (self_keep) return DREG_EINVAL;
         const dim3 g1(CG / BNS_COLS, B);
         float* sums = sums_keep ? sums_keep : coef;
 #define BNS_BWD(Tt, NRv) hipLaunchKernelGGL((bn_small_bwd_kernel<Tt, NRv>), g1, dim3(256), 0, st, (const Tt*)x, (const Tt*)dy, (const Tt*)y, scale_shift, mean_rstd, \
@@ -1939,12 +2148,24 @@
         return DREG_OK;
     }
     if (B > BN_MAX_GRIDS || slabs_ragged(CG)) return DREG_EINVAL;
+    if (self_keep && (!deferred || (g_bn_debug_skip & 2) || !dreg_bn_self_coef_supported(B, V, C, dtype))) return DREG_EINVAL;
     dim3 grid(nch, B, slabs);
     const int g_stored = (dres && relu && y && dres != dy && dres != dx && g_bn_store_g && !(g_bn_debug_skip & 2)) ? 1 : 0;
     if (g_bn_debug_skip & 2) {}
     else if (dtype == 0) hipLaunchKernelGGL((bn_partial_kernel<bf16_t, 1>), grid, dim3(256), 0, st, (const bf16_t*)x, (const bf16_t*)dy, (const bf16_t*)y, mean_rstd, workspace, V, C, rpc, relu, scale_shift, g_stored ? (bf16_t*)dres : nullptr);
     else hipLaunchKernelGGL((bn_partial_kernel<float, 1>), grid, dim3(256), 0, st, (const float*)x, (const float*)dy, (const float*)y, mean_rstd, workspace, V, C, rpc, relu, scale_shift, g_stored ? (float*)dres : nullptr);
     DREG_LAUNCH_CHECK();
+    if (self_keep) {
+        const int rows = bn_self_rows(B, V, C, G);
+        const dim3 sgrid((V + rows - 1) / rows, B, bn_self_slabs(C, G));
+        if (dtype == 0) hipLaunchKernelGGL((bn_bwd_apply_self_kernel<bf16_t, 4>), sgrid, dim3(256), 0, st, (const bf16_t*)x, (const bf16_t*)dy, (const bf16_t*)y, workspace, mean_rstd, scale_shift,
+                                           (bf16_t*)dx, (bf16_t*)dres, self_keep, V, C, nch, rows, relu, g_stored);
+        else hipLaunchKernelGGL((bn_bwd_apply_self_kernel<float, 4>), sgrid, dim3(256), 0, st, (const float*)x, (const float*)dy, (const float*)y, workspace, mean_rstd, scale_shift,
+                                (float*)dx, (float*)dres, self_keep, V, C, nch, rows, relu, g_stored);
+        DREG_LAUNCH_CHECK();
+        *deferred = 1;
+        return DREG_OK;
+    }
     hipLaunchKernelGGL(bn_bwd_finalize_kernel, dim3(C), dim3(64 * (B < 8 ? B : 8)), 0, st, workspace, coef, dgamma, dbeta, B, nch, C, V, accumulate);
     DREG_LAUNCH_CHECK();
     const size_t tg = (size_t)B * V * CG;
diff --git a/dreg_nerf_amd/lib.py b/dreg_nerf_amd/lib.py
--- a/dreg_nerf_amd/lib.py
+++ b/dreg_nerf_amd/lib.py
@@ -96,6 +96,11 @@
     "dreg_bn3d_bwd_defer_params": (I, [P] * 11 + [I, I, I, I, I, I, P, P, P]),
     "dreg_bn_running_update_batched": (I, [P, I, I, I, F, P]),
     "dreg_bn_param_grad_batched": (I, [P, I, I, I, I, P]),
+    "dreg_bn_self_coef_supported": (I, [I, I, I, I]),
+    "dreg_bn_self_coef_use": (I, [I, I, I, I, I]),
+    "dreg_bn_self_coef_rows": (I, [I, I, I, I]),
+    "dreg_bn3d_fwd_self_coef": (I, [P, P, P, P, P, P, P, P, I, I, I, I, F, I, I, P, P, P]),
+    "dreg_bn3d_bwd_self_coef": (I, [P, P, P, P, P, P, P, P, I, I, I, I, I, P, P]),
     "dreg_maxpool3d_fwd": (I, [P, P, P] + [I] * 9 + [P]),
     "dreg_maxpool3d_bwd": (I, [P, P, P] + [I] * 9 + [P]),
     "dreg_maxpool3d_bwd_acc": (I, [P, P, P] + [I] * 10 + [P]),
@@ -131,6 +136,7 @@
     "dreg_exec_destroy": (None, [P]),
     "dreg_exec_op_halo": (I, [P, I]),
     "dreg_exec_op_pointwise": (I, [P, I]),
+    "dreg_exec_op_bn_self_coef": (I, [P, I]),
     "dreg_exec_op_wgrad_grouped": (I, [P, I]),
     "dreg_exec_arena_bytes": (Z, [P]),
     "dreg_exec_pack_bytes": (Z, [P]),
@@ -297,6 +303,7 @@
     "dreg_conv3_halo64_set": (None, [I]),
     "dreg_conv3_halo_set_prof": (None, [P]),
     "dreg_bn_set_small_max_voxels": (None, [I]),
+    "dreg_bn_set_self_wgs": (None, [I]),
     "dreg_ngp_set_rgb_chunks": (None, [I]),
     "dreg_ngp_set_density_unroll": (None, [I]),
     "dreg_ngp_set_xcd_levels": (None, [I]),
@@ -317,7 +324,7 @@
 
 class ExecOpts(ctypes.Structure):
     _fields_ = [(n, c_int) for n in ("sparse_grads", "bn_batch_tails", "fuse_stem", "sparse_stem", "fold_res_bn", "fold_splitk", "group_wgrad",
-                                     "s2_accumulate", "fuse_bn_stats", "brick", "defer_head_pg", "persistent_deep", "guard", "pointwise_stream")] + [("reserved", c_int * 2)]
+                                     "s2_accumulate", "fuse_bn_stats", "brick", "defer_head_pg", "persistent_deep", "guard", "pointwise_stream", "bn_self_coef")] + [("reserved", c_int * 1)]
 
 
 SCENE_MAX_BLOCKS = 4
diff --git a/include/dreg_nerf.h b/include/dreg_nerf.h
--- a/include/dreg_nerf.h
+++ b/include/dreg_nerf.h
@@ -142,6 +142,14 @@
 int dreg_bn_small_in_regs(int B, int V, int C, int dtype);
 int dreg_bn_running_update_batched(const void* descs_dev, int n, int block_base, int nblocks, float momentum, void* stream);
 int dreg_bn_param_grad_batched(const void* descs_dev, int n, int block_base, int nblocks, int accumulate, void* stream);
+int dreg_bn_self_coef_supported(int B, int V, int C, int dtype);
+int dreg_bn_self_coef_use(int B, int V, int C, int dtype, int backward);
+int dreg_bn_self_coef_rows(int B, int V, int C, int dtype);
+int dreg_bn3d_fwd_self_coef(const void* x, const void* res, void* y, const float* gamma, const float* beta, float* scale_shift, float* mean_rstd,
+                            float* sums, int rows_per_chunk, int B, int V, int C, float eps, int relu, int dtype, double* keep,
+                            const float* res_scale_shift, void* stream);
+int dreg_bn3d_bwd_self_coef(const void* x, const void* dy, const void* y, const float* scale_shift, const float* mean_rstd,
+                            void* dx, void* dres, float* workspace, int B, int V, int C, int relu, int dtype, double* keep, void* stream);
 
 int dreg_bn_relu_maxpool_fwd(const void* x, void* pooled, uint8_t* argmax, const float* gamma, const float* beta,
                              float* running_mean, float* running_var, float* scale_shift, float* mean_rstd, float* workspace,
@@ -235,7 +243,8 @@
     int persistent_deep;
     int guard;
     int pointwise_stream;
-    int reserved[2];
+    int bn_self_coef;
+    int reserved[1];
 } dreg_exec_opts;
 void dreg_exec_default_opts(dreg_exec_opts* o);
 void* dreg_exec_create_opts(const int* tensors, int nt, const int* ops, int nops, const int64_t* params, int np, const dreg_exec_opts* opts);
@@ -255,6 +264,7 @@
 int dreg_exec_repack(void* h, const void* descs_dev, const int* row_desc_dev, void* stream);
 int dreg_exec_op_halo(void* h, int op);
 int dreg_exec_op_wgrad_grouped(void* h, int op);
+int dreg_exec_op_bn_self_coef(void* h, int op);
 int dreg_exec_op_pointwise(void* h, int op);
 void dreg_exec_set_overlap(void* h, int enable);
 void dreg_exec_set_input_row_occupancy(void* h, const uint8_t* rowocc);
diff --git a/include/dreg_nerf_probe.h b/include/dreg_nerf_probe.h
--- a/include/dreg_nerf_probe.h
+++ b/include/dreg_nerf_probe.h
@@ -24,6 +24,7 @@
 void dreg_conv_set_glds_stages(int stages);
 void dreg_conv_set_wgrad_target_blocks(int blocks);
 void dreg_bn_set_small_max_voxels(int v);
+void dreg_bn_set_self_wgs(int n);
 void dreg_sstem_set_pool_blocks(int n);
 void dreg_voxel_set_own_sort(int on);
 void dreg_conv_set_bn_stats_epilogue(int on);
```

Result: faster. 266.1 pairs/s, median of 6 (+1.0%).
